# SuperScientificSoftwareLaboratory/DASP

Measured on AMD Instinct MI355X. Metric: SpMV GFLOP/s (f64), higher is better.
Workload: dtype f64; 1 GPU; HV15R synthetic stand-in (seeded; SuiteSparse dims/row statistics), A=1, x=1; rows=2017169, cols=2017169, nnz=275454726, partition=single GPU, generator_rev=26e32ff958e7, y_candidates=1

## Files before the change

### dasp_amd/_lib.py

```python
import ctypes as C
import os
import subprocess

_HERE = os.path.dirname(os.path.abspath(__file__))
SO_PATH = os.environ.get("DASP_AMD_SO") or os.path.join(_HERE, "libdasp_amd.so")


class DaspError(RuntimeError):
    def __init__(self, status, msg):
        super().__init__("dasp status %d: %s" % (status, msg))
        self.status = status


class Options(C.Structure):
    _fields_ = [
        ("threshold", C.c_double), ("block_longest", C.c_int), ("y_order", C.c_int), ("long_piece", C.c_int),
        ("host_threads", C.c_int), ("n_parts", C.c_int), ("part_bounds", C.POINTER(C.c_int)), ("part_stride", C.c_int),
        ("x_window", C.c_int), ("row_window", C.c_int), ("cid16", C.c_int), ("stream_policy", C.c_int),
        ("col_panels", C.c_int), ("slab_max_len", C.c_int), ("x_window_hybrid", C.c_int), ("piece_min_len", C.c_int),
        ("chunk_pairs", C.c_int), ("cid8", C.c_int), ("short_seg", C.c_int), ("row_tile_max", C.c_int), ("sort_columns", C.c_int),
        ("two_phase", C.c_int), ("tp_col_block", C.c_int), ("tp_row_block", C.c_int), ("long_cb", C.c_int),
        ("value_map", C.c_int),
    ]


class Stats(C.Structure):
    _fields_ = [(n, C.c_int) for n in (
        "precision rowA colA nnzA short_row_1 common_13 short_row_3 short_row_4 short_row_2 row_long row_block "
        "row_zero nnz_short nnz_long origin_nnz_reg nnz_irreg rowloop").split()] + [
        ("fill0_nnz_short", C.c_longlong), ("fill0_nnz_long", C.c_longlong), ("fill0_nnz_reg", C.c_longlong),
        ("rate_fill0", C.c_double), ("data_X", C.c_longlong), ("data_origin1", C.c_longlong),
        ("n_med_blocks", C.c_int), ("n_long_pieces", C.c_int), ("n_long_multi", C.c_int), ("n_short_tiles", C.c_int),
        ("n_workgroups", C.c_int), ("pre_ms", C.c_double),
        ("x_window_on", C.c_int), ("n_windows", C.c_int), ("n_windows_lds", C.c_int), ("lds_bytes", C.c_int),
        ("row_window", C.c_int), ("window_nnz_frac", C.c_double), ("cid16_on", C.c_int),
        ("n_col_panels", C.c_int), ("x_window_hybrid", C.c_int), ("med_rows_as_pieces", C.c_int), ("chunk_pairs", C.c_int), ("cid8_chunks", C.c_int), ("short_seg", C.c_int),
        ("row_tile_max", C.c_int), ("n_row_tiles", C.c_int), ("row_tile_nnz", C.c_longlong),
        ("two_phase", C.c_int), ("tp_col_block", C.c_int), ("tp_row_blocks", C.c_int), ("tp_units", C.c_int), ("tp_segments", C.c_longlong), ("tp_seg_elems", C.c_int),
        ("lcb_rows", C.c_int), ("lcb_col_block", C.c_int), ("lcb_units", C.c_int), ("lcb_elems", C.c_longlong),
        ("ref_fill0_nnz_short", C.c_longlong), ("ref_fill0_nnz_long", C.c_longlong), ("ref_fill0_nnz_reg", C.c_longlong), ("ref_data_X", C.c_longlong),
        ("ref_nnz_irreg", C.c_int), ("ref_origin_nnz_reg", C.c_int), ("ref_blocknum", C.c_int), ("ref_warp_number", C.c_int), ("ref_rate_fill0", C.c_double)]

    def as_dict(self):
        return {n: getattr(self, n) for n, _ in self._fields_}


class MgInfo(C.Structure):
    _fields_ = [(n, C.c_int) for n in "precision n_gpus rank rowA colA row_begin row_end stride".split()] + [
        ("nnz_own", C.c_longlong), ("nnz_other", C.c_longlong), ("overlap", C.c_int), ("has_comm", C.c_int), ("square", C.c_int), ("stream_memops", C.c_int), ("fused_step", C.c_int), ("exchange", C.c_int)]

    def as_dict(self):
        return {n: getattr(self, n) for n, _ in self._fields_}


def build(force=False):
    src = os.path.join(_HERE, "csrc")
    if force:
        subprocess.check_call(["make", "-C", src, "-s", "clean"])
    subprocess.check_call(["make", "-C", src, "-s", "-j8", "all"])
    return SO_PATH


_lib = None


def _preload_hip_runtime():
    import importlib.util
    import sys
    if "torch" in sys.modules:
        return
    try:
        spec = importlib.util.find_spec("torch")
    except (ImportError, ValueError):
        spec = None
    if spec is None or not spec.origin:
        return
    cand = os.path.join(os.path.dirname(spec.origin), "lib", "libamdhip64.so")
    if os.path.exists(cand):
        try:
            C.CDLL(cand, mode=C.RTLD_GLOBAL)
        except OSError:
            pass


def lib():
    global _lib
    if _lib is not None:
        return _lib
    if not os.path.exists(SO_PATH):
        raise ImportError(
            "dasp_amd: %s is missing. Build it with `python -c 'import __graft_entry__ as g; g.build()'` "
            "(hipcc --offload-arch=gfx950). There is no fallback implementation." % SO_PATH)
    _preload_hip_runtime()
    L = C.CDLL(SO_PATH)
    ip, vp = C.POINTER(C.c_int), C.c_void_p
    L.dasp_last_error.restype = C.c_char_p
    L.dasp_version.restype = C.c_char_p
    L.dasp_free.argtypes = [vp]
    L.dasp_options_default.argtypes = [C.POINTER(Options)]
    L.dasp_mmio_allinone_f64.argtypes = [ip, ip, ip, ip, C.POINTER(ip), C.POINTER(ip), C.POINTER(C.POINTER(C.c_double)), C.c_char_p]
    L.dasp_mmio_allinone_f16.argtypes = [ip, ip, ip, ip, C.POINTER(ip), C.POINTER(ip), C.POINTER(C.POINTER(C.c_uint16)), C.c_char_p]
    L.dasp_csr_save.argtypes = [C.c_char_p, C.c_int, C.c_int, C.c_int, C.c_int, C.c_int, vp, vp, vp]
    L.dasp_csr_load.argtypes = [C.c_char_p, C.c_int, ip, ip, ip, ip, C.POINTER(ip), C.POINTER(ip), C.POINTER(vp)]
    L.dasp_plan_create.argtypes = [C.POINTER(vp), C.c_int, C.c_int, C.c_int, C.c_int, vp, vp, vp, C.POINTER(Options)]
    L.dasp_plan_create_device.argtypes = [C.POINTER(vp), C.c_int, C.c_int, C.c_int, C.c_int, vp, vp, vp, C.POINTER(Options)]
    L.dasp_plan_download_array.argtypes = [vp, C.c_char_p, vp, C.c_size_t]
    L.dasp_plan_destroy.argtypes = [vp]
    L.dasp_plan_save.argtypes = [vp, C.c_char_p]
    L.dasp_plan_load.argtypes = [C.POINTER(vp), C.c_char_p]
    L.dasp_plan_order.argtypes = [vp]
    L.dasp_plan_order.restype = ip
    L.dasp_plan_stats.argtypes = [vp, C.POINTER(Stats)]
    L.dasp_plan_y_order.argtypes = [vp]
    L.dasp_plan_x_len.argtypes = [vp]
    L.dasp_plan_x_len.restype = C.c_longlong
    L.dasp_plan_host_array.argtypes = [vp, C.c_char_p, C.POINTER(vp), ip]
    L.dasp_plan_host_array.restype = C.c_longlong
    L.dasp_plan_panel_count.argtypes = [vp]
    L.dasp_plan_panel.argtypes = [vp, C.c_int]
    L.dasp_plan_panel.restype = vp
    L.dasp_plan_panel_range.argtypes = [vp, C.c_int, ip, ip]
    L.dasp_plan_upload.argtypes = [vp]
    L.dasp_plan_drop_host.argtypes = [vp]
    L.dasp_plan_update_values.argtypes = [vp, vp, vp]
# ... 67 lines not shown
```

### dasp_amd/api.py

```python
import ctypes as C
import os

import numpy as np

from . import _lib
from ._lib import DaspError, Options, Stats

Y_PERMUTED, Y_NATURAL = 0, 1


def _vp(a):
    return a.ctypes.data_as(C.c_void_p)


def _dtype(precision):
    if precision == 64:
        return np.float64
    if precision == 16:
        return np.float16
    raise ValueError("precision must be 64 or 16")


def mmio_allinone(filename, precision=64):
    L = _lib.lib()
    ip = C.POINTER(C.c_int)
    m, n, nnz, sym = C.c_int(), C.c_int(), C.c_int(), C.c_int()
    rp, ci = ip(), ip()
    if precision == 64:
        v = C.POINTER(C.c_double)()
        rc = L.dasp_mmio_allinone_f64(C.byref(m), C.byref(n), C.byref(nnz), C.byref(sym), C.byref(rp), C.byref(ci), C.byref(v), os.fsencode(filename))
    else:
        v = C.POINTER(C.c_uint16)()
        rc = L.dasp_mmio_allinone_f16(C.byref(m), C.byref(n), C.byref(nnz), C.byref(sym), C.byref(rp), C.byref(ci), C.byref(v), os.fsencode(filename))
    _lib.check(rc)
    k = nnz.value
    row_ptr = np.ctypeslib.as_array(rp, (m.value + 1,)).copy()
    col_idx = np.ctypeslib.as_array(ci, (max(k, 1),))[:k].copy()
    raw = np.ctypeslib.as_array(v, (max(k, 1),))[:k].copy()
    val = raw if precision == 64 else raw.view(np.float16)
    for q in (rp, ci, v):
        L.dasp_free(C.cast(q, C.c_void_p))
    return m.value, n.value, k, sym.value, row_ptr, col_idx, val


def csr_save(path, row_ptr, col_idx, val, n_cols, is_symmetric=0, precision=64):
    rp = np.ascontiguousarray(row_ptr, np.int32)
    ci = np.ascontiguousarray(col_idx, np.int32)
    v = np.ascontiguousarray(val, _dtype(precision))
    _lib.check(_lib.lib().dasp_csr_save(os.fsencode(path), precision, rp.size - 1, int(n_cols), int(ci.size), int(is_symmetric), _vp(rp), _vp(ci), _vp(v)))


def csr_load(path, precision=64):
    L = _lib.lib()
    ip = C.POINTER(C.c_int)
    m, n, nnz, sym = C.c_int(), C.c_int(), C.c_int(), C.c_int()
    rp, ci, v = ip(), ip(), C.c_void_p()
    _lib.check(L.dasp_csr_load(os.fsencode(path), precision, C.byref(m), C.byref(n), C.byref(nnz), C.byref(sym), C.byref(rp), C.byref(ci), C.byref(v)))
    k = nnz.value
    row_ptr = np.ctypeslib.as_array(rp, (m.value + 1,)).copy()
    col_idx = np.ctypeslib.as_array(ci, (max(k, 1),))[:k].copy()
    ct = C.c_double if precision == 64 else C.c_uint16
    raw = np.ctypeslib.as_array(C.cast(v, C.POINTER(ct)), (max(k, 1),))[:k].copy()
    val = raw if precision == 64 else raw.view(np.float16)
    for q in (C.cast(rp, C.c_void_p), C.cast(ci, C.c_void_p), v):
        L.dasp_free(q)
    return m.value, n.value, k, sym.value, row_ptr, col_idx, val


class Plan:

    def __init__(self, csrRowPtr, csrColIdx, csrVal, colA, precision=64, threshold=0.75, block_longest=256,
                 y_order=Y_PERMUTED, long_piece=0, host_threads=0, part_bounds=None, part_stride=0, x_window=0, row_window=0, cid16=0, stream_policy=0,
                 col_panels=0, slab_max_len=0, x_window_hybrid=0, piece_min_len=0, chunk_pairs=0, cid8=0, short_seg=0, row_tile_max=0, sort_columns=0,
                 two_phase=0, tp_col_block=0, tp_row_block=0, long_cb=0, value_map=0):
        L = _lib.lib()
        self.precision = precision
        dt = _dtype(precision)
        rp = np.ascontiguousarray(csrRowPtr, np.int32)
        ci = np.ascontiguousarray(csrColIdx, np.int32)
        v = np.ascontiguousarray(csrVal, dt)
        self.rowA, self.colA, self.nnzA = rp.size - 1, int(colA), int(ci.size)
        opt = Options()
        L.dasp_options_default(C.byref(opt))
        opt.threshold, opt.block_longest, opt.y_order = threshold, block_longest, y_order
        opt.long_piece, opt.host_threads = long_piece, host_threads
        opt.x_window, opt.row_window, opt.cid16, opt.stream_policy = x_window, row_window, cid16, stream_policy
        opt.col_panels, opt.slab_max_len, opt.x_window_hybrid, opt.piece_min_len = col_panels, slab_max_len, x_window_hybrid, piece_min_len
        opt.chunk_pairs, opt.cid8, opt.short_seg, opt.row_tile_max, opt.sort_columns = chunk_pairs, cid8, short_seg, row_tile_max, sort_columns
        opt.two_phase, opt.tp_col_block, opt.tp_row_block, opt.long_cb = two_phase, tp_col_block, tp_row_block, long_cb
        opt.value_map = value_map
        self._pb = None
        if part_bounds is not None:
            self._pb = np.ascontiguousarray(part_bounds, np.int32)
            opt.n_parts = self._pb.size - 1
            opt.part_bounds = self._pb.ctypes.data_as(C.POINTER(C.c_int))
            opt.part_stride = int(part_stride)
        self._h = C.c_void_p()
        _lib.check(L.dasp_plan_create(C.byref(self._h), precision, self.rowA, self.colA, self.nnzA, _vp(rp), _vp(ci), _vp(v), C.byref(opt)))
        self.y_order = y_order
        self.x_len = self.colA if part_bounds is None else (self._pb.size - 1) * int(part_stride)

    @classmethod
    def from_device(cls, d_row_ptr, d_col_idx, d_val, rowA, colA, nnzA, precision=64, threshold=0.75, block_longest=256,
                    y_order=Y_PERMUTED, long_piece=0, part_bounds=None, part_stride=0, x_window=0, row_window=0, cid16=0, col_panels=0, slab_max_len=0,
                    x_window_hybrid=0, piece_min_len=0, chunk_pairs=0, cid8=0, short_seg=0, row_tile_max=0, sort_columns=0, two_phase=0, tp_col_block=0, tp_row_block=0, long_cb=0,
                    value_map=0):
        L = _lib.lib()
        self = cls.__new__(cls)
        self.precision, self.rowA, self.colA, self.nnzA = precision, int(rowA), int(colA), int(nnzA)
        opt = Options()
        L.dasp_options_default(C.byref(opt))
        opt.threshold, opt.block_longest, opt.y_order, opt.long_piece = threshold, block_longest, y_order, long_piece
        opt.x_window, opt.row_window, opt.cid16, opt.col_panels = x_window, row_window, cid16, col_panels
        opt.slab_max_len, opt.x_window_hybrid, opt.piece_min_len = slab_max_len, x_window_hybrid, piece_min_len
        opt.chunk_pairs, opt.cid8, opt.short_seg, opt.row_tile_max, opt.sort_columns = chunk_pairs, cid8, short_seg, row_tile_max, sort_columns
        opt.two_phase, opt.tp_col_block, opt.tp_row_block, opt.long_cb = two_phase, tp_col_block, tp_row_block, long_cb
        opt.value_map = value_map
        self._pb = None
        if part_bounds is not None:
            self._pb = np.ascontiguousarray(part_bounds, np.int32)
            opt.n_parts, opt.part_stride = self._pb.size - 1, int(part_stride)
            opt.part_bounds = self._pb.ctypes.data_as(C.POINTER(C.c_int))
        self._h = C.c_void_p()
        _lib.check(L.dasp_plan_create_device(C.byref(self._h), precision, self.rowA, self.colA, self.nnzA, C.c_void_p(d_row_ptr),
                                             C.c_void_p(d_col_idx), C.c_void_p(d_val), C.byref(opt)))
        self.y_order = y_order
        self.x_len = int(L.dasp_plan_x_len(self._h))
        return self

    def device_array(self, name, count, dtype):
        out = np.empty(count, dtype)
        _lib.check(_lib.lib().dasp_plan_download_array(self._h, name.encode(), _vp(out), out.nbytes))
        return out

    def save(self, path):
        _lib.check(_lib.lib().dasp_plan_save(self._h, os.fsencode(path)))

    @classmethod
    def load(cls, path):
        self = cls.__new__(cls)
        self._h = C.c_void_p()
        self._pb = None
        _lib.check(_lib.lib().dasp_plan_load(C.byref(self._h), os.fsencode(path)))
        st = self.stats
        self.precision, self.rowA, self.colA, self.nnzA = st["precision"], st["rowA"], st["colA"], st["nnzA"]
        self.y_order = _lib.lib().dasp_plan_y_order(self._h)
        self.x_len = int(_lib.lib().dasp_plan_x_len(self._h))
        return self

    @property
    def order_rid(self):
        if self.rowA == 0:
            return np.zeros(0, np.int32)
        p = _lib.lib().dasp_plan_order(self._h)
        return np.ctypeslib.as_array(p, (max(self.rowA, 1),))[: self.rowA].copy()

    @property
    def stats(self):
        s = Stats()
        _lib.check(_lib.lib().dasp_plan_stats(self._h, C.byref(s)))
        return s.as_dict()

    @property
    def n_panels(self):
        return int(_lib.lib().dasp_plan_panel_count(self._h))

    def panel(self, k):
        L = _lib.lib()
        h = L.dasp_plan_panel(self._h, k)
        if not h:
            raise _lib.DaspError(-10, L.dasp_last_error().decode("utf-8", "replace"))
        b, e = C.c_int(), C.c_int()
        _lib.check(L.dasp_plan_panel_range(self._h, k, C.byref(b), C.byref(e)))
        sub = Plan.__new__(Plan)
        sub._h, sub._pb, sub._borrowed, sub._parent = C.c_void_p(h), None, True, self
        st = sub.stats
        sub.precision, sub.rowA, sub.colA, sub.nnzA = st["precision"], st["rowA"], st["colA"], st["nnzA"]
        sub.y_order, sub.x_len = Y_NATURAL, st["colA"]
        return sub, b.value, e.value

    def host_array(self, name):
        ptr, eb = C.c_void_p(), C.c_int()
        n = _lib.lib().dasp_plan_host_array(self._h, name.encode(), C.byref(ptr), C.byref(eb))
        if n < 0:
            _lib.check(int(n))
        if name in ("med_cid16", "long_cid16", "rt_start", "tp_lrow", "tp_lcol", "lcb_lcol"):
            dt = np.uint16
        elif name.endswith("_val_map"):
            dt = np.uint32
        elif name == "rt_mask":
            dt = np.uint64
        elif name == "med_cid8":
            dt = np.uint8
        elif eb.value == 4:
            dt = np.int32
        else:
            dt = np.float64 if eb.value == 8 else np.float16
        if n == 0:
            return np.zeros(0, dt)
        buf = (C.c_char * (n * eb.value)).from_address(ptr.value)
# ... 137 lines not shown
```

### dasp_amd/csrc/device.hpp

```cpp
#pragma once

#include <cstddef>
#include <vector>

#include "plan.hpp"

namespace dasp {

struct ShortDev {
    int len, count, tiles, tile0;
    long long elem_off;
    SlotMap map;
    int seg, rpt;
};

struct DevArgs {
    const void *x;
    void *y;
    const void *long_val; const int *long_cid; const int *piece_ptr; const int *piece_dst; void *partial;
    const int *multi_ptr; const int *multi_dst;
    int n_pieces, n_multi;
    int pair_mode;
    const int *med_ptr; const void *med_val; const int *med_cid;
    const unsigned short *med_cid16; const int *med_base;
    const unsigned char *med_cid8; const int *med_c8ptr;
    const int *irr_ptr; const void *irr_val; const int *irr_cid;
    int n_blocks, row_block, row_long;
    const int *med_dst; const int *win_cmin; const int *win_len;
    int n_windows, blocks_per_win;
    int win_hybrid;
    int win_xcd;
    int win_rel16;
    int ywt;
    int skip0;
    int acc;
    int wpw;
    const void *short_val; const int *short_cid; const ShortDev *groups;
    int n_short_tiles;
    int short_tpw, n_short_waves;
    int grp_wave0[kNumShortGroups];
    int grp_tile0[kNumShortGroups];
    const int *order;
    int wg_long, wg_med, wg_short;
    int xcd_on;
    int xcd_blk[9];
    int med_stride;
    const void *rt_val; const int *rt_cid; const int *rt_ptr; const unsigned short *rt_start; const unsigned long long *rt_mask;
    int n_rt_tiles, wg_rt, rt_max;
    const unsigned short *long_cid16; const int *long_base; const int *piece_c16;
    const int *med_nt;
    int wg_rot;
    int win_tiles;
};

struct TpDev {
    const unsigned short *lcol; const int *dst; const int *unit;
    const void *val; const unsigned short *lrow; void *xs;
    const int *rb_row0; const int *rb_seg0;
    int n_units, n_rb, cb, rb_max, xlen, m;
};

struct LcbDev {
    const void *val; const unsigned short *lcol; const int *ptr; const int *unit; const int *row_dst; void *partial;
    int n_units, n_rows, n_cb, cb, xlen;
};

struct ArenaMap {
    size_t long_val = 0, long_cid = 0, med_val = 0, med_cid = 0, med_cid16 = 0, med_cid8 = 0, med_base = 0, irr_val = 0, irr_cid = 0,
           short_val = 0, short_cid = 0, rt_val = 0, rt_cid = 0, long_cid16 = 0, long_base = 0, piece_c16 = 0;
};

struct DevicePlan {
    void *dargs = nullptr;
    void *args_sent = nullptr;
    void *arena = nullptr;
    size_t arena_bytes = 0;
    ArenaMap map{};
    DevArgs args{};
    TpDev tp{};
    LcbDev lcb{};
    bool nt = false;
    bool win1 = false;
    bool seven_waves = false;
    bool long16 = false;
    int device = -1;
    size_t ypart_stride = 0;
    void *vm_map = nullptr, *vm_runs = nullptr;
    bool vm_ready = false;
    void *pk_map[7] = {};
    int vm_n_runs = 0;
    long long vm_blocks = 0, vm_slots = 0;
    std::vector<Plan *> vm_arenas;
};
int value_map_upload(Plan &p);
void value_map_free(DevicePlan *d);


int require_device();
int upload_plan(Plan &p);
void choose_long16(Plan &p);
int sync_dev_args(Plan &p);
int upload_plan_unpacked(Plan &p);
int launch_spmv(Plan &p, const void *dX, void *dY, void *stream, bool accumulate);
int spmv_kernel_allow_full_lds(int precision, bool c16);
int tp_kernels_allow_lds();
int spmv_kernel_f16_resident(bool c16);
int tune_placement(Plan &p, int trials, const void *dX, void *dY, double *ms_first, double *ms_kept);

constexpr size_t kMgWordGathered = 20480, kMgWordOwnGo = 20480 + 4096, kMgWordReady = 20480 + 8192, kMgWordErr = 20480 + 12288, kMgWordXcd = 40960, kMgWordBytes = 40960 + 2048;
struct MgStepCtl {
    void *words;
    unsigned long long need;
    unsigned long long step;
    const void *mark; const void *mark_members;
    const void *blk_order;
    int n_marked, n_mark_shards;
    int max_pollers;
    int poll_sleep;
    long long timeout_ticks;
    double poll_at;
    void *err;
    int ready_by_event;
};
bool mg_step_supported(const Plan &own, const Plan *other);
void mg_step_marks(const Plan &own, const unsigned char *has_other, std::vector<unsigned char> &mark, std::vector<int> &blk_order, double hot_at = -1.0);
int launch_mg_step(Plan &own, Plan *other, const void *x_own, const void *x_gathered, void *y, const MgStepCtl &c, void *stream);
int mg_step_resident_per_cu();
struct MgStep2Ctl {
    const void *wg_list; const void *blk_order;
    int n_push, n_free, n_marked, n_total, max_pollers;
    const void *arrived; int world, rank;
    unsigned long long need;
    void *err; long long timeout_ticks; int poll_sleep;
    int fence_mode;
    void *xcd_fenced; unsigned long long step;
};
struct MgPushArgs;
int launch_mg_step2(Plan &plan, const void *x, void *y, const MgStep2Ctl &c, const MgPushArgs &push, void *stream);
int launch_mg_wait(const void *word, unsigned long long need, long long timeout_ticks, void *err, void *stream);
int launch_mg_flag(void *word, unsigned long long value, void *stream);

}
```

### dasp_amd/csrc/devpack.hip

```cpp
#include <hip/hip_runtime.h>
#include <hipcub/hipcub.hpp>

#include <memory>
#include <thread>

#include <algorithm>
#include <chrono>
#include <cstdio>
#include <cstdlib>
#include <cstring>
#include <string>
#include <type_traits>
#include <vector>

#include "device.hpp"

namespace dasp {

#define HIP_TRYP(expr)                                                                         \
    do {                                                                                       \
        hipError_t e_ = (expr);                                                                \
        if (e_ != hipSuccess) {                                                                \
            set_error(std::string(#expr) + ": " + hipGetErrorString(e_));                      \
            return e_ == hipErrorNoDevice ? DASP_ERR_NO_DEVICE : DASP_ERR_HIP;                 \
// ... 928 lines not shown
    unsigned *lmap = nullptr;
    if (p.value_map) {
        HIP_TRYP(hipMalloc(&dp.pk_map[6], L.elems * 4));
        lmap = static_cast<unsigned *>(dp.pk_map[6]);
        HIP_TRYP(hipMemset(lmap, 0, L.elems * 4));
    }
    if (s.n > 0) {
        if (vb == 8)
            hipLaunchKernelGGL((k_lcb_fill<unsigned long long>), dim3(grid_for(s.n)), dim3(256), 0, 0, s.keys, s.idx, s.n, s.start, dp.lcb.ptr, L.n_rows(), L.cb, d.ci,
                               static_cast<const unsigned long long *>(d.val), d.src, lcol, static_cast<unsigned long long *>(lval), lmap);
        else
            hipLaunchKernelGGL((k_lcb_fill<unsigned short>), dim3(grid_for(s.n)), dim3(256), 0, 0, s.keys, s.idx, s.n, s.start, dp.lcb.ptr, L.n_rows(), L.cb, d.ci,
                               static_cast<const unsigned short *>(d.val), d.src, lcol, static_cast<unsigned short *>(lval), lmap);
        HIP_TRYP(hipGetLastError());
    }
    HIP_TRYP(hipDeviceSynchronize());
    return DASP_OK;
}

int devpack_finish_two_phase(Plan &p, const DevCsr &d, const DevTiles &tp, const std::vector<long long> &off2, const std::vector<long long> &off1, const DevTiles &lcb)
{
    FormScratch sc;
    const size_t n_tiles = off1.size(), S = p.tp.segments;
    const int *d_off2 = nullptr, *d_off1 = nullptr;
    if (S > 0) {
        std::vector<int> h(off2.begin(), off2.end());
        if (int rc = form_upload(sc, h.data(), h.size(), &d_off2)) return rc;
        h.assign(off1.begin(), off1.end());
        if (int rc = form_upload(sc, h.data(), h.size(), &d_off1)) return rc;
    }
    if (int rc = upload_plan_unpacked(p)) return rc;
    DevicePlan &dp = *p.dev;
    if (S > 0) {
        auto *lcol = const_cast<unsigned short *>(dp.tp.lcol), *lrow = const_cast<unsigned short *>(dp.tp.lrow);
        auto *tval = static_cast<unsigned short *>(const_cast<void *>(dp.tp.val));
        HIP_TRYP(hipMemset(lcol, 0, S * kTpSeg * 2));
        HIP_TRYP(hipMemset(lrow, 0xFF, S * kTpSeg * 2));
        HIP_TRYP(hipMemset(tval, 0, S * kTpSeg * 2));
        unsigned *tmap = nullptr;
        if (p.value_map) {
            HIP_TRYP(hipMalloc(&dp.pk_map[5], S * kTpSeg * 4));
            tmap = static_cast<unsigned *>(dp.pk_map[5]);
            HIP_TRYP(hipMemset(tmap, 0, S * kTpSeg * 4));
        }
        const int n_cb = std::max(1, (p.n + p.tp.cb - 1) / p.tp.cb);
        if (tp.n > 0) hipLaunchKernelGGL(k_tp_fill, dim3(grid_for(tp.n)), dim3(256), 0, 0, tp.keys, tp.idx, tp.n, tp.start, d_off2, d_off1, n_cb, p.tp.cb, d.ci,
                                         static_cast<const unsigned short *>(d.val), d.src, lcol, lrow, tval, tmap);
        HIP_TRYP(hipGetLastError());
        hipLaunchKernelGGL(k_tp_dst, dim3(grid_for((long long)S)), dim3(256), 0, 0, d_off2, d_off1, (int)n_tiles, (int)S, const_cast<int *>(dp.tp.dst));
        HIP_TRYP(hipGetLastError());
    }
    if (int rc = lcb_fill(p, d, lcb)) return rc;
    HIP_TRYP(hipDeviceSynchronize());
    p.host_dropped = true;
    if (p.value_map) return value_map_upload(p);
    return DASP_OK;
}

int devpack_finish_panels_lcb(Plan &p, const DevCsr &d, const DevTiles &lcb)
{
    if (int rc = upload_plan_unpacked(p)) return rc;
    if (int rc = lcb_fill(p, d, lcb)) return rc;
    p.host_dropped = true;
    if (p.value_map) return value_map_upload(p);
    return DASP_OK;
}

int devpack_finish_panels(Plan &p) { return upload_plan(p); }
int devpack_fetch_csr(const Plan &p, const DevCsr &d, int *ci, void *val)
{
    if (p.nnz <= 0) return DASP_OK;
    HIP_TRYP(hipMemcpy(ci, d.ci, (size_t)p.nnz * sizeof(int), hipMemcpyDeviceToHost));
    if (val) HIP_TRYP(hipMemcpy(val, d.val, (size_t)p.nnz * (size_t)p.geo.vbytes, hipMemcpyDeviceToHost));
    return DASP_OK;
}
int devpack_current_device() { int d = 0; if (hipGetDevice(&d) != hipSuccess) { (void)hipGetLastError(); d = 0; } return d; }
void devpack_use_device(int device) { if (device >= 0) (void)hipSetDevice(device); }

int devpack_all(Plan &p, const DevCsr &d, const PackMeta &m)
{
    if (int rc = upload_plan_unpacked(p)) return rc;
    const int rc = p.precision == 64 ? pack_all_typed<double>(p, d, m) : pack_all_typed<_Float16>(p, d, m);
    if (rc == DASP_OK) p.host_dropped = true;
    if (rc == DASP_OK && p.value_map && !p.panel) return value_map_upload(p);
    return rc;
}

__global__ void k_spin_us(long long ticks)
{
    const long long t0 = wall_clock64();
    while (wall_clock64() - t0 < ticks) __builtin_amdgcn_s_sleep(8);
}
__global__ void __launch_bounds__(256) k_spin_fat(long long ticks, int *sink)
{
    __shared__ int pad[19744 / 4];
    asm volatile("v_mov_b32 v255, 0" ::: "v255");
    asm volatile("v_accvgpr_write_b32 a23, 0" ::: "a23");
    pad[threadIdx.x] = (int)ticks;
    const long long t0 = wall_clock64();
    while (wall_clock64() - t0 < ticks) __builtin_amdgcn_s_sleep(8);
    if (ticks < 0) sink[threadIdx.x] = pad[255 - threadIdx.x];
}
int devpack_spin(void *stream, int micros, int channels)
{
    if (micros <= 0) return DASP_OK;
    if (channels > 0) hipLaunchKernelGGL(k_spin_fat, dim3(channels), dim3(256), 0, static_cast<hipStream_t>(stream), (long long)micros * 100, (int *)nullptr);
    else hipLaunchKernelGGL(k_spin_us, dim3(1), dim3(64), 0, static_cast<hipStream_t>(stream), (long long)micros * 100);
    HIP_TRYP(hipGetLastError());
    return DASP_OK;
}

namespace {

struct ValueRun { long long dst_off, map_off, count, blk0; int arena, pad; };
constexpr int kRefreshMaxArenas = 65;
constexpr int kRefreshThreads = 256, kRefreshSteps = 4;
struct RefreshBases { char *base[kRefreshMaxArenas]; };
template <int VB> struct RefreshGeo { static constexpr int G = VB == 8 ? 4 : 8; };
__host__ __device__ constexpr long long refresh_slots_per_block(int vb) { return (long long)kRefreshThreads * kRefreshSteps * (vb == 8 ? 4 : 8); }

typedef unsigned int vm_u32x4 __attribute__((ext_vector_type(4)));
typedef unsigned long long vm_u64x2 __attribute__((ext_vector_type(2)));

template <class V, bool NT> __device__ __forceinline__ V vm_load(const V *p) { if constexpr (NT) return __builtin_nontemporal_load(p); else return *p; }
template <class V, bool NT> __device__ __forceinline__ void vm_store(V *p, V v) { if constexpr (NT) __builtin_nontemporal_store(v, p); else *p = v; }

template <int VB, bool NT>
__global__ void __launch_bounds__(kRefreshThreads) dasp_value_refresh_kernel(const ValueRun *__restrict__ runs, int n_runs, const unsigned int *__restrict__ map,
                                                                           const void *__restrict__ src, RefreshBases bases)
{
    using W = std::conditional_t<VB == 8, unsigned long long, unsigned short>;
    constexpr int G = RefreshGeo<VB>::G;
    const long long b = blockIdx.x;
    int lo = 0, hi = n_runs - 1;
    while (lo < hi) { const int mid = (lo + hi + 1) >> 1; if (runs[mid].blk0 <= b) lo = mid; else hi = mid - 1; }
    const long long count = runs[lo].count, e_blk = (b - runs[lo].blk0) * refresh_slots_per_block(VB);
    W *dst = reinterpret_cast<W *>(bases.base[runs[lo].arena] + runs[lo].dst_off);
    const unsigned int *mp = map + runs[lo].map_off;
    const W *s = static_cast<const W *>(src);
#pragma unroll
    for (int step = 0; step < kRefreshSteps; ++step) {
        const long long e = e_blk + ((long long)step * kRefreshThreads + threadIdx.x) * G;
        if (e + G <= count) {
            unsigned int ix[G];
            const vm_u32x4 m0 = vm_load<vm_u32x4, NT>(reinterpret_cast<const vm_u32x4 *>(mp + e));
            ix[0] = m0.x; ix[1] = m0.y; ix[2] = m0.z; ix[3] = m0.w;
            if constexpr (G == 8) {
                const vm_u32x4 m1 = vm_load<vm_u32x4, NT>(reinterpret_cast<const vm_u32x4 *>(mp + e + 4));
                ix[4] = m1.x; ix[5] = m1.y; ix[6] = m1.z; ix[7] = m1.w;
            }
            W v[G];
#pragma unroll
            for (int i = 0; i < G; ++i) v[i] = ix[i] ? s[ix[i] - 1u] : (W)0;
            if constexpr (VB == 8) {
                vm_store<vm_u64x2, NT>(reinterpret_cast<vm_u64x2 *>(dst + e), vm_u64x2{v[0], v[1]});
                vm_store<vm_u64x2, NT>(reinterpret_cast<vm_u64x2 *>(dst + e + 2), vm_u64x2{v[2], v[3]});
            } else {
                vm_u32x4 o;
                o.x = (unsigned)v[0] | ((unsigned)v[1] << 16); o.y = (unsigned)v[2] | ((unsigned)v[3] << 16);
                o.z = (unsigned)v[4] | ((unsigned)v[5] << 16); o.w = (unsigned)v[6] | ((unsigned)v[7] << 16);
                vm_store<vm_u32x4, NT>(reinterpret_cast<vm_u32x4 *>(dst + e), o);
            }
        } else if (e < count) {
            for (long long j = e; j < count; ++j) { const unsigned int ix = mp[j]; dst[j] = ix ? s[ix - 1u] : (W)0; }
        }
    }
}
// ... 112 lines not shown
    const char *s = static_cast<const char *>(val);
    const int T = resolve_threads(p.opt.host_threads);
    for (const HostRun &r : hr) {
        char *dst = r.host_val->data();
        const uint32_t *mp = r.map->data();
        const size_t n = r.count, per = std::max<size_t>(1 << 16, (n + (size_t)T - 1) / (size_t)T);
        std::vector<std::thread> th;
        auto work = [&](size_t b, size_t e) {
            for (size_t j = b; j < e; ++j) { if (mp[j]) std::memcpy(dst + j * vb, s + (size_t)(mp[j] - 1) * vb, vb); else std::memset(dst + j * vb, 0, vb); }
        };
        for (size_t b = per; b < n; b += per) th.emplace_back(work, b, std::min(n, b + per));
        work(0, std::min(n, per));
        for (auto &t : th) t.join();
    }
}

static int value_map_usable(const Plan &p)
{
    if (p.panel) { set_error("a column panel is refreshed through its parent plan (dasp_plan_update_values on the parent)"); return DASP_ERR_ARG; }
    if (p.loaded) { set_error("a plan loaded from a file carries no value map (plan files do not store one): create the plan with value_map = 1"); return DASP_ERR_STATE; }
    if (!p.value_map) { set_error("the plan has no value map: create it with dasp_options_t::value_map = 1"); return DASP_ERR_STATE; }
    return DASP_OK;
}

}

extern "C" {

int dasp_plan_update_values(dasp_plan_t *plan, const void *dVal, void *stream)
{
    using namespace dasp;
    if (!plan || (!dVal && plan->impl.nnz > 0)) { set_error("dasp_plan_update_values: NULL argument"); return DASP_ERR_ARG; }
    Plan &p = plan->impl;
    if (int rc = value_map_usable(p)) return rc;
    if (!p.dev) { set_error("dasp_plan_update_values: the plan is not uploaded (dasp_plan_upload, or dasp_plan_update_values_host for host values)"); return DASP_ERR_STATE; }
    if (!p.dev->vm_ready) { set_error("dasp_plan_update_values: the plan's value map did not reach the device (its upload failed): upload the plan again"); return DASP_ERR_STATE; }
    if (!p.host_dropped) if (int rc = dasp_plan_drop_host(plan)) return rc;
    return value_refresh_launch(p, dVal, static_cast<hipStream_t>(stream));
}

int dasp_plan_update_values_host(dasp_plan_t *plan, const void *csrVal)
{
    using namespace dasp;
    if (!plan || (!csrVal && plan->impl.nnz > 0)) { set_error("dasp_plan_update_values_host: NULL argument"); return DASP_ERR_ARG; }
    Plan &p = plan->impl;
    if (int rc = value_map_usable(p)) return rc;
    if (p.dev && !p.dev->vm_ready) { set_error("dasp_plan_update_values_host: the plan's value map did not reach the device (its upload failed): upload the plan again"); return DASP_ERR_STATE; }
    try {
        if (!p.host_dropped) value_refresh_host(p, csrVal);
    } catch (const std::exception &e) { set_error(std::string("dasp_plan_update_values_host: ") + e.what()); return DASP_ERR_NOMEM; }
    if (p.dev && p.dev->vm_blocks > 0) {
        const size_t bytes = (size_t)p.nnz * (size_t)p.geo.vbytes;
        void *stage = nullptr;
        HIP_TRYP(hipDeviceSynchronize());
        HIP_TRYP(hipMalloc(&stage, std::max<size_t>(bytes, 16)));
        hipError_t e = hipMemcpy(stage, csrVal, bytes, hipMemcpyHostToDevice);
        int rc = e == hipSuccess ? value_refresh_launch(p, stage, nullptr) : DASP_ERR_HIP;
        if (e != hipSuccess) set_error(std::string("dasp_plan_update_values_host: staging copy: ") + hipGetErrorString(e));
        if (rc == DASP_OK && (e = hipStreamSynchronize(nullptr)) != hipSuccess) { set_error(std::string("dasp_plan_update_values_host: ") + hipGetErrorString(e)); rc = DASP_ERR_HIP; }
        (void)hipFree(stage);
        return rc;
    }
    return DASP_OK;
}

long long dasp_plan_value_map_slots(const dasp_plan_t *plan)
{
    using namespace dasp;
    if (!plan) return DASP_ERR_ARG;
    const Plan &p = plan->impl;
    if (!p.value_map || p.loaded) return 0;
    if (p.host_dropped) return p.dev ? p.dev->vm_slots : 0;
    std::vector<HostRun> hr;
    collect_runs(const_cast<Plan &>(p), hr);
    long long n = 0;
    for (const HostRun &r : hr) n += (long long)r.count;
    return n;
}

}

namespace dasp {

int download_array(Plan &p, const char *name, void *dst, size_t bytes)
{
    if (!p.dev || !p.dev->arena) { set_error("plan not on the device"); return DASP_ERR_STATE; }
    const ArenaMap &mp = p.dev->map;
    const size_t vb = (size_t)p.geo.vbytes;
    if (std::strcmp(name, "lcb_val") == 0 && p.dev->lcb.val) {
        if (bytes != p.lcb.elems * vb) { set_error("size mismatch for lcb_val"); return DASP_ERR_ARG; }
        if (bytes) HIP_TRYP(hipMemcpy(dst, p.dev->lcb.val, bytes, hipMemcpyDeviceToHost));
        return DASP_OK;
    }
    if (std::strcmp(name, "lcb_lcol") == 0 && p.dev->lcb.lcol) {
        if (bytes != p.lcb.elems * 2) { set_error("size mismatch for lcb_lcol"); return DASP_ERR_ARG; }
        if (bytes) HIP_TRYP(hipMemcpy(dst, p.dev->lcb.lcol, bytes, hipMemcpyDeviceToHost));
        return DASP_OK;
    }
    if (p.two_phase) {
        const TpDev &q = p.dev->tp;
        const size_t S = p.tp.segments;
        struct { const char *n; const void *ptr; size_t len; } tt[] = {
            {"tp_lcol", q.lcol, S * kTpSeg * 2}, {"tp_dst", q.dst, S * 4}, {"tp_val", q.val, S * kTpSeg * vb}, {"tp_lrow", q.lrow, S * kTpSeg * 2}, {"tp_xs", q.xs, S * kTpSeg * vb}};
        for (auto &t : tt)
            if (std::strcmp(t.n, name) == 0) {
                if (bytes != t.len) { set_error(std::string("size mismatch for ") + name); return DASP_ERR_ARG; }
                if (t.len) HIP_TRYP(hipMemcpy(dst, t.ptr, t.len, hipMemcpyDeviceToHost));
                return DASP_OK;
            }
        set_error(std::string("unknown device array of a two-phase plan: ") + name);
        return DASP_ERR_ARG;
    }
    struct { const char *n; size_t off, len; } tab[] = {
        {"long_val", mp.long_val, p.cnt_long * vb}, {"long_cid", mp.long_cid, p.cnt_long * 4}, {"long_cid16", mp.long_cid16, p.cnt_long * 2}, {"long_base", mp.long_base, p.cnt_long_chunks * 4},
        {"med_val", mp.med_val, p.cnt_reg * vb}, {"med_cid", mp.med_cid, p.cid16 ? 0 : p.cnt_reg * 4},
        {"med_cid16", mp.med_cid16, p.cid16 ? (p.cnt_reg - p.cnt_reg8) * 2 : 0}, {"med_cid8", mp.med_cid8, p.cnt_reg8}, {"med_base", mp.med_base, p.cid16 ? (size_t)p.med_ptr.back() * 4 : 0},
        {"irr_val", mp.irr_val, p.cnt_irr * vb}, {"irr_cid", mp.irr_cid, p.cnt_irr * 4},
        {"short_val", mp.short_val, p.cnt_short * vb}, {"short_cid", mp.short_cid, p.cnt_short * 4},
        {"rt_val", mp.rt_val, p.cnt_rt * vb}, {"rt_cid", mp.rt_cid, p.cnt_rt * 4},
    };
    for (auto &t : tab)
        if (std::strcmp(t.n, name) == 0) {
            if (bytes != t.len) { set_error(std::string("size mismatch for ") + name); return DASP_ERR_ARG; }
            if (t.len) HIP_TRYP(hipMemcpy(dst, static_cast<char *>(p.dev->arena) + t.off, t.len, hipMemcpyDeviceToHost));
            return DASP_OK;
        }
    set_error(std::string("unknown device array: ") + name);
    return DASP_ERR_ARG;
}

}
```

### dasp_amd/csrc/kernels.hip

```cpp
#include <hip/hip_runtime.h>

#include <chrono>
#include <thread>
#include <cmath>
#include <cstdint>
#include <cstdio>
#include <cstdlib>
#include <cstring>
#include <string>
#include <vector>

#include "plan.hpp"
#include "device.hpp"

#include "spmv_device.hpp"

namespace dasp {
#ifdef DASP_STAMPS
extern int g_stamp_launch;
#endif

template <class T, bool NT, bool C16, bool WIN, bool C8 = false, int MW = 0, bool L16 = false>
__global__ __launch_bounds__(WIN ? 1024 : 256, WIN ? kMinWavesWin : MW ? MW : kMinWavesPlain) void dasp_spmv_kernel(CallArgs c)
{
    extern __shared__ __attribute__((aligned(16))) char lds_raw[];
#ifdef DASP_STAMPS
    Stamps st; st.begin(c.stamp_launch);
#else
    Stamps st; st.begin(0);
#endif
    const DevArgs a = load_args(c);
    static_assert(!L16 || (!WIN && !C8 && MW == 0), "the 16-bit long ids ride in the plain build only");
    spmv_body<T, NT, C16, WIN, C8, false, WIN, L16>(a, lds_raw, blockIdx.x, st);
#ifdef DASP_STAMPS
    st.finish(a.wpw);
#endif
}

template <class T, bool NT, bool C16>
__global__ __launch_bounds__(256, sizeof(T) == 2 ? 7 : kMinWavesPlain) void dasp_spmv_rt_kernel(CallArgs c)
{
    extern __shared__ __attribute__((aligned(16))) char lds_raw[];
#ifdef DASP_STAMPS
    Stamps st; st.begin(c.stamp_launch);
#else
    Stamps st; st.begin(0);
#endif
    const DevArgs a = load_args(c);
    spmv_body<T, NT, C16, false, false, true>(a, lds_raw, blockIdx.x, st);
}

template <class T, bool C16>
__global__ __launch_bounds__(1024, 4) void dasp_spmv_win1_kernel(CallArgs c)
{
    extern __shared__ __attribute__((aligned(16))) char lds_raw[];
#ifdef DASP_STAMPS
    Stamps st; st.begin(c.stamp_launch);
#else
    Stamps st; st.begin(0);
#endif
    const DevArgs a = load_args(c);
    spmv_body<T, true, C16, true, false>(a, lds_raw, blockIdx.x, st);
#ifdef DASP_STAMPS
    st.finish(a.wpw);
#endif
}

constexpr int kMaxMergedPanels = 8;
struct PanelCall {
    const DevArgs *plan[kMaxMergedPanels];
    int wg_end[kMaxMergedPanels];
    const void *x; char *part; size_t stride_bytes; int np;
};
__device__ __forceinline__ CallArgs panel_of(const PanelCall &c, int &wg)
{
    int k = 0, first = 0;
    const DevArgs *p = c.plan[0];
#pragma unroll
    for (int i = 1; i < kMaxMergedPanels; ++i) {
        const bool in = i < c.np && (int)blockIdx.x >= c.wg_end[i - 1];
        k = in ? i : k; first = in ? c.wg_end[i - 1] : first; p = in ? c.plan[i] : p;
    }
    wg = (int)blockIdx.x - first;
#ifdef DASP_STAMPS
    return CallArgs{p, c.x, c.part + (size_t)k * c.stride_bytes, 0, 0, -1};
#else
    return CallArgs{p, c.x, c.part + (size_t)k * c.stride_bytes, 0, 0};
#endif
}
template <class T, bool NT, bool C16>
__global__ __launch_bounds__(256, sizeof(T) == 2 ? 7 : kMinWavesPlain) void dasp_spmv_panels_kernel(PanelCall c)
{
    extern __shared__ __attribute__((aligned(16))) char lds_raw[];
    int wg;
    const CallArgs ca = panel_of(c, wg);
    Stamps st; st.begin(0);
    const DevArgs a = load_args(ca);
    spmv_body<T, NT, C16, false, false, true>(a, lds_raw, wg, st);
}

template <class T>
__global__ __launch_bounds__(256) void dasp_long_reduce_kernel(CallArgs c)
{
    const DevArgs a = load_args(c);
    using part_t = typename Tr<T>::part_t;
    __shared__ part_t wsum[kWavesPerWG];
    const int lane = threadIdx.x & 63, wave = threadIdx.x >> 6;
    const int i = blockIdx.x;
    const int q0 = a.multi_ptr[i], q1 = a.multi_ptr[i + 1];
    const part_t *part = static_cast<const part_t *>(a.partial);
    part_t s0 = 0, s1 = 0, s2 = 0, s3 = 0;
    int q = q0 + (int)threadIdx.x;
    for (; q + 768 < q1; q += 1024) { s0 += part[q]; s1 += part[q + 256]; s2 += part[q + 512]; s3 += part[q + 768]; }
    for (; q < q1; q += 256) s0 += part[q];
    const part_t s = wave_sum((s0 + s1) + (s2 + s3));
    if (lane == 0) wsum[wave] = s;
// ... 233 lines not shown
    acc = __builtin_amdgcn_mfma_f64_16x16x4f64(A, B, acc, 0, 0, 0);
    for (int r = 0; r < 4; ++r) D[((l >> 4) + 4 * r) * 16 + (l & 15)] = acc[r];
}
__global__ void selftest_f16_kernel(float *D)
{
    const int l = threadIdx.x;
    f16x4 A, B;
    for (int j = 0; j < 4; ++j) {
        const int k = 4 * (l >> 4) + j;
        A[j] = (_Float16)(float)(((l & 15) + 2 * k) % 7 + 1);
        B[j] = (_Float16)(float)((3 * k + (l & 15)) % 5 + 1);
    }
    f32x4 acc = {0, 0, 0, 0};
    acc = __builtin_amdgcn_mfma_f32_16x16x16f16(A, B, acc, 0, 0, 0);
    for (int r = 0; r < 4; ++r) D[(4 * (l >> 4) + r) * 16 + (l & 15)] = acc[r];
}


#define HIP_TRY(expr)                                                                          \
    do {                                                                                       \
        hipError_t e_ = (expr);                                                                \
        if (e_ != hipSuccess) {                                                                \
            set_error(std::string(#expr) + ": " + hipGetErrorString(e_));                      \
            return e_ == hipErrorNoDevice ? DASP_ERR_NO_DEVICE : DASP_ERR_HIP;                 \
        }                                                                                      \
    } while (0)


int spmv_kernel_allow_full_lds(int precision, bool c16)
{
    const int bytes = kWinLdsMax;
    hipError_t e1, e2;
#define DASP_ATTR(TT, NTV, CV) hipFuncSetAttribute(reinterpret_cast<const void *>(&dasp_spmv_kernel<TT, NTV, CV, true>), hipFuncAttributeMaxDynamicSharedMemorySize, bytes)
    if (precision == 64) { e1 = c16 ? DASP_ATTR(double, true, true) : DASP_ATTR(double, true, false); e2 = c16 ? DASP_ATTR(double, false, true) : DASP_ATTR(double, false, false); }
    else { e1 = c16 ? DASP_ATTR(_Float16, true, true) : DASP_ATTR(_Float16, true, false); e2 = c16 ? DASP_ATTR(_Float16, false, true) : DASP_ATTR(_Float16, false, false); }
#undef DASP_ATTR
    HIP_TRY(e1);
    HIP_TRY(e2);
    if (precision == 64) HIP_TRY(c16 ? hipFuncSetAttribute(reinterpret_cast<const void *>(&dasp_spmv_win1_kernel<double, true>), hipFuncAttributeMaxDynamicSharedMemorySize, bytes)
                                     : hipFuncSetAttribute(reinterpret_cast<const void *>(&dasp_spmv_win1_kernel<double, false>), hipFuncAttributeMaxDynamicSharedMemorySize, bytes));
    else HIP_TRY(c16 ? hipFuncSetAttribute(reinterpret_cast<const void *>(&dasp_spmv_win1_kernel<_Float16, true>), hipFuncAttributeMaxDynamicSharedMemorySize, bytes)
                     : hipFuncSetAttribute(reinterpret_cast<const void *>(&dasp_spmv_win1_kernel<_Float16, false>), hipFuncAttributeMaxDynamicSharedMemorySize, bytes));
    return DASP_OK;
}
int spmv_kernel_f16_resident(bool c16)
{
    const void *fn = c16 ? reinterpret_cast<const void *>(&dasp_spmv_kernel<_Float16, true, true, false>)
                         : reinterpret_cast<const void *>(&dasp_spmv_kernel<_Float16, true, false, false>);
    int fit = 0;
    if (hipOccupancyMaxActiveBlocksPerMultiprocessor(&fit, fn, kWave * kWavesPerWG, 0) != hipSuccess) fit = 0;
    (void)hipGetLastError();
    return fit;
}

template <class T>
static int launch_typed(Plan &p, const DevArgs &a, hipStream_t s)
{
    const int grid = a.wg_long + a.wg_med + a.wg_short + a.wg_rt;
    const bool nt = p.dev->nt;
    if (int rc = sync_dev_args(p)) return rc;
#ifdef DASP_STAMPS
    const CallArgs c{static_cast<const DevArgs *>(p.dev->dargs), a.x, a.y, a.acc, a.ywt, g_stamp_launch >= 0 ? g_stamp_launch++ : -1};
#else
    const CallArgs c{static_cast<const DevArgs *>(p.dev->dargs), a.x, a.y, a.acc, a.ywt};
#endif
    if (a.wg_rt > 0) {
        const size_t lds = (size_t)kWavesPerWG * kRowTile * (size_t)a.rt_max * sizeof(typename Tr<T>::part_t);
        if (nt && p.cid16) hipLaunchKernelGGL((dasp_spmv_rt_kernel<T, true, true>), dim3(grid), dim3(256), lds, s, c);
        else if (nt) hipLaunchKernelGGL((dasp_spmv_rt_kernel<T, true, false>), dim3(grid), dim3(256), lds, s, c);
        else if (p.cid16) hipLaunchKernelGGL((dasp_spmv_rt_kernel<T, false, true>), dim3(grid), dim3(256), lds, s, c);
        else hipLaunchKernelGGL((dasp_spmv_rt_kernel<T, false, false>), dim3(grid), dim3(256), lds, s, c);
    } else if (grid > 0) {
        const size_t lds = p.windowed ? (size_t)p.lds_bytes : 0;
        const bool c16 = p.cid16;
#define DASP_FOR_EACH(M) \
        if (nt && c16 && p.windowed) { M(true, true, true); } else if (nt && c16) { M(true, true, false); } \
        else if (nt && p.windowed) { M(true, false, true); } else if (nt) { M(true, false, false); } \
        else if (c16 && p.windowed) { M(false, true, true); } else if (c16) { M(false, true, false); } \
        else if (p.windowed) { M(false, false, true); } else { M(false, false, false); }
#define DASP_LAUNCH(NTV, CV, WINV) hipLaunchKernelGGL((dasp_spmv_kernel<T, NTV, CV, WINV>), dim3(grid), dim3(kWave * a.wpw), lds, s, c)
        if (p.windowed && p.dev->win1 && !nt) {
            if (c16) hipLaunchKernelGGL((dasp_spmv_win1_kernel<T, true>), dim3(grid), dim3(kWave * a.wpw), lds, s, c);
            else hipLaunchKernelGGL((dasp_spmv_win1_kernel<T, false>), dim3(grid), dim3(kWave * a.wpw), lds, s, c);
        } else if (sizeof(T) == 8 && c16 && !p.windowed && p.cnt_reg8 > 0) {
            if (p.dev->seven_waves) {
                if (nt) hipLaunchKernelGGL((dasp_spmv_kernel<double, true, true, false, true, 7>), dim3(grid), dim3(kWave * a.wpw), lds, s, c);
                else hipLaunchKernelGGL((dasp_spmv_kernel<double, false, true, false, true, 7>), dim3(grid), dim3(kWave * a.wpw), lds, s, c);
            }
            else if (nt) hipLaunchKernelGGL((dasp_spmv_kernel<double, true, true, false, true>), dim3(grid), dim3(kWave * a.wpw), lds, s, c);
            else hipLaunchKernelGGL((dasp_spmv_kernel<double, false, true, false, true>), dim3(grid), dim3(kWave * a.wpw), lds, s, c);
        } else if (!p.windowed && p.dev->long16 && !(sizeof(T) == 8 && p.dev->seven_waves)) {
            if (nt && c16) hipLaunchKernelGGL((dasp_spmv_kernel<T, true, true, false, false, 0, true>), dim3(grid), dim3(kWave * a.wpw), lds, s, c);
            else if (nt) hipLaunchKernelGGL((dasp_spmv_kernel<T, true, false, false, false, 0, true>), dim3(grid), dim3(kWave * a.wpw), lds, s, c);
            else if (c16) hipLaunchKernelGGL((dasp_spmv_kernel<T, false, true, false, false, 0, true>), dim3(grid), dim3(kWave * a.wpw), lds, s, c);
            else hipLaunchKernelGGL((dasp_spmv_kernel<T, false, false, false, false, 0, true>), dim3(grid), dim3(kWave * a.wpw), lds, s, c);
        } else if (sizeof(T) == 8 && !p.windowed && p.dev->seven_waves) {
            if (nt && c16) hipLaunchKernelGGL((dasp_spmv_kernel<double, true, true, false, false, 7>), dim3(grid), dim3(kWave * a.wpw), lds, s, c);
            else if (nt) hipLaunchKernelGGL((dasp_spmv_kernel<double, true, false, false, false, 7>), dim3(grid), dim3(kWave * a.wpw), lds, s, c);
            else if (c16) hipLaunchKernelGGL((dasp_spmv_kernel<double, false, true, false, false, 7>), dim3(grid), dim3(kWave * a.wpw), lds, s, c);
            else hipLaunchKernelGGL((dasp_spmv_kernel<double, false, false, false, false, 7>), dim3(grid), dim3(kWave * a.wpw), lds, s, c);
        } else
        DASP_FOR_EACH(DASP_LAUNCH)
#undef DASP_LAUNCH
#undef DASP_FOR_EACH
    }
    if (a.n_multi > 0)
        hipLaunchKernelGGL((dasp_long_reduce_kernel<T>), dim3(a.n_multi), dim3(256), 0, s, c);
    HIP_TRY(hipGetLastError());
    return DASP_OK;
}

int set_stream_policy(Plan &p, int policy)
{
    if (policy < 0 || policy > 2) { set_error("stream_policy must be 0, 1 or 2"); return DASP_ERR_ARG; }
    p.opt.stream_policy = policy;
    if (p.dev) p.dev->nt = policy == 2 || (policy != 1 && p.stats.data_X > kStreamBytes);
    const int sub = policy != 0 ? policy : (p.stats.data_X > kStreamBytes ? 2 : 1);
    for (auto &h : p.panels) if (int rc = set_stream_policy(h->impl, sub)) return rc;
    return DASP_OK;
}

int tp_kernels_allow_lds()
{
    HIP_TRY(hipFuncSetAttribute(reinterpret_cast<const void *>(&dasp_tp_expand_kernel<_Float16>), hipFuncAttributeMaxDynamicSharedMemorySize, 160 * 1024));
    HIP_TRY(hipFuncSetAttribute(reinterpret_cast<const void *>(&dasp_tp_reduce_kernel<_Float16>), hipFuncAttributeMaxDynamicSharedMemorySize, 160 * 1024));
    HIP_TRY(hipFuncSetAttribute(reinterpret_cast<const void *>(&dasp_lcb_kernel<_Float16>), hipFuncAttributeMaxDynamicSharedMemorySize, 160 * 1024));
    HIP_TRY(hipFuncSetAttribute(reinterpret_cast<const void *>(&dasp_lcb_kernel<double>), hipFuncAttributeMaxDynamicSharedMemorySize, 160 * 1024));
    return DASP_OK;
}

template <class T>
static int launch_panels_merged_typed(Plan &p, const void *dX, char *part, size_t stride_bytes, hipStream_t s)
{
    const int np = (int)p.panels.size();
    PanelCall c{}, r{};
    c.x = dX; c.part = part; c.stride_bytes = stride_bytes; c.np = np;
    int grid = 0, grid2 = 0, rt_max = 0;
    const Plan &p0 = p.panels[0]->impl;
    for (int k = 0; k < np; ++k) {
        Plan &q = p.panels[(size_t)k]->impl;
        if (!q.dev || !q.dev->arena || q.windowed || q.two_phase || !q.panels.empty() || q.cnt_reg8 > 0 || q.cid16 != p0.cid16 || q.dev->nt != p0.dev->nt || q.dev->args.med_stride != p0.dev->args.med_stride) return 1;
        if (int rc = sync_dev_args(q)) return rc;
        const DevArgs &a = q.dev->args;
        grid += a.wg_long + a.wg_med + a.wg_short + a.wg_rt;
        grid2 += (a.n_multi + kWavesPerWG - 1) / kWavesPerWG;
        rt_max = std::max(rt_max, a.wg_rt > 0 ? a.rt_max : 0);
        c.plan[k] = static_cast<const DevArgs *>(q.dev->dargs); c.wg_end[k] = grid;
        r.plan[k] = c.plan[k]; r.wg_end[k] = grid2;
    }
    r.x = dX; r.part = part; r.stride_bytes = stride_bytes; r.np = np;
    const size_t lds = (size_t)kWavesPerWG * kRowTile * (size_t)rt_max * sizeof(typename Tr<T>::part_t);
    const bool nt = p0.dev->nt, c16 = p0.cid16;
    if (grid > 0) {
        if (nt && c16) hipLaunchKernelGGL((dasp_spmv_panels_kernel<T, true, true>), dim3(grid), dim3(256), lds, s, c);
        else if (nt) hipLaunchKernelGGL((dasp_spmv_panels_kernel<T, true, false>), dim3(grid), dim3(256), lds, s, c);
        else if (c16) hipLaunchKernelGGL((dasp_spmv_panels_kernel<T, false, true>), dim3(grid), dim3(256), lds, s, c);
        else hipLaunchKernelGGL((dasp_spmv_panels_kernel<T, false, false>), dim3(grid), dim3(256), lds, s, c);
    }
    if (grid2 > 0) hipLaunchKernelGGL((dasp_long_reduce_panels_kernel<T>), dim3(grid2), dim3(256), 0, s, r);
    HIP_TRY(hipGetLastError());
    return DASP_OK;
}
static int launch_panels_merged(Plan &p, const void *dX, char *part, size_t stride_bytes, hipStream_t s)
{
    static const bool off = [] { const char *e = std::getenv("DASP_PANELS_MERGED"); return e && std::atoi(e) == 0; }();
    if (off || p.panels.empty() || p.panels.size() > (size_t)kMaxMergedPanels) return 1;
// ... 195 lines not shown
```

### dasp_amd/csrc/multigpu.cpp

```cpp
#include <hip/hip_runtime_api.h>
#include <hip/hip_ext.h>
#include <rccl/rccl.h>

#include <dlfcn.h>

#include <algorithm>
#include <chrono>
#include <cstdlib>
#include <cstring>
#include <exception>
#include <memory>
#include <mutex>
#include <new>
#include <string>
#include <thread>
#include <vector>

#include <unistd.h>

#include "plan.hpp"
#include "device.hpp"
#include "mgx.hpp"

using namespace dasp;
// ... 187 lines not shown
    std::vector<void *> fake_peers;
    ncclComm_t comm = nullptr;

    size_t vb() const { return precision == 64 ? 8 : 2; }
    size_t all_bytes() const { return (size_t)stride * vb() * (size_t)world; }
    bool one_stream() const { return step2 && fused && push; }
    char *gcur() const { return static_cast<char *>(yg) + (one_stream() ? (size_t)(k2 & 1) * all_bytes() : push ? (size_t)(xseq & 1) * all_bytes() : 0); }
    int rows() const { return bounds[(size_t)rank + 1] - bounds[(size_t)rank]; }
    ~dasp_mg_plan()
    {
        if (device >= 0) (void)hipSetDevice(device);
        if (cs) (void)hipStreamSynchronize(cs);
        if (device >= 0) (void)hipDeviceSynchronize();
        if (comm && rccl()->CommDestroy) (void)rccl()->CommDestroy(comm);
        for (size_t r = 0; r < peer_opened.size(); ++r)
            if (peer_opened[r]) { if (peer_gather[r]) (void)hipIpcCloseMemHandle(peer_gather[r]); if (peer_flags[r]) (void)hipIpcCloseMemHandle(peer_flags[r]); }
        for (void *p : {xflags, d_push_dst, d_push_count, push_scratch, d_wg_list, d_push_dst2, d_push_count2}) if (p) (void)hipFree(p);
        if (ev_y) (void)hipEventDestroy(ev_y);
        if (ev_g) (void)hipEventDestroy(ev_g);
        for (hipEvent_t e : ev_x) if (e) (void)hipEventDestroy(e);
        if (err_word) (void)hipHostFree(err_word);
        if (cs) (void)hipStreamDestroy(cs);
        if (rs) (void)hipStreamDestroy(rs);
        for (uint64_t *w : sig) if (w) (void)hipFree(w);
        if (words) (void)hipFree(words);
        if (d_mark) (void)hipFree(d_mark);
        if (d_blk_order) (void)hipFree(d_blk_order);
        for (void *p : {ys[0], yg}) if (p) (void)hipFree(p);
        if (xg && xg != yg) (void)hipFree(xg);
        if (own) dasp_plan_destroy(own);
        if (other) dasp_plan_destroy(other);
    }
};

namespace {

template <class T>
void split_by_owner(int m, const int *rp, const int *ci, const T *val, int lo, int hi, int threads,
                    std::vector<int> &rpO, std::vector<int> &ciO, std::vector<T> &vO,
                    std::vector<int> &rpR, std::vector<int> &ciR, std::vector<T> &vR)
{
    rpO.assign((size_t)m + 1, 0); rpR.assign((size_t)m + 1, 0);
    auto par = [&](auto f) {
        const int parts = std::max(1, std::min(threads, m / 4096 + 1));
        std::vector<std::thread> th;
        for (int t = 0; t < parts; ++t) {
            const int b = (int)((long long)m * t / parts), e = (int)((long long)m * (t + 1) / parts);
            th.emplace_back([=] { f(b, e); });
        }
        for (auto &x : th) x.join();
    };
    par([&](int b, int e) {
        for (int i = b; i < e; ++i) {
            int o = 0;
            for (int j = rp[i]; j < rp[i + 1]; ++j) o += ci[j] >= lo && ci[j] < hi;
            rpO[(size_t)i + 1] = o; rpR[(size_t)i + 1] = rp[i + 1] - rp[i] - o;
        }
    });
    for (int i = 0; i < m; ++i) { rpO[(size_t)i + 1] += rpO[i]; rpR[(size_t)i + 1] += rpR[i]; }
    ciO.resize((size_t)rpO[m]); vO.resize((size_t)rpO[m]); ciR.resize((size_t)rpR[m]); vR.resize((size_t)rpR[m]);
    par([&](int b, int e) {
        for (int i = b; i < e; ++i) {
            int o = rpO[i], r = rpR[i];
            for (int j = rp[i]; j < rp[i + 1]; ++j) {
                if (ci[j] >= lo && ci[j] < hi) { ciO[(size_t)o] = ci[j] - lo; vO[(size_t)o++] = val[j]; }
                else { ciR[(size_t)r] = ci[j]; vR[(size_t)r++] = val[j]; }
            }
        }
    });
}

template <class T>
int create_impl(dasp_mg_plan &g, const int *rp, const int *ci, const T *val, const dasp_options_t *user)
{
    const int m = g.rows();
    const int lo = g.bounds[(size_t)g.rank], hi = g.bounds[(size_t)g.rank + 1];
    dasp_options_t opt;
    if (user) opt = *user; else dasp_options_default(&opt);
    opt.y_order = DASP_Y_NATURAL;
    opt.short_seg = -1;
    opt.two_phase = -1;
    opt.n_parts = 0; opt.part_bounds = nullptr; opt.part_stride = 0;
    opt.value_map = 0;
    const int nnz = rp[m];
    if (!g.square) {
        g.nnz_own = nnz; g.nnz_other = 0;
        return dasp_plan_create(&g.own, g.precision, m, g.colA, nnz, rp, ci, val, &opt);
    }
    dasp_options_t part = opt;
    part.n_parts = g.world; part.part_bounds = g.bounds.data(); part.part_stride = g.stride;
    if (!g.overlap) {
        g.nnz_own = nnz; g.nnz_other = 0;
        return dasp_plan_create(&g.own, g.precision, m, g.colA, nnz, rp, ci, val, &part);
    }
    if (g.step2) {
        std::vector<unsigned char> has((size_t)std::max(m, 1), 0);
        long long other = 0;
        for (int i = 0; i < m; ++i) {
            int o = 0;
            for (int j = rp[i]; j < rp[i + 1]; ++j) o += !(ci[j] >= lo && ci[j] < hi);
            has[(size_t)i] = o > 0; other += o;
        }
        g.nnz_own = nnz - other; g.nnz_other = other;
        if (int rc = dasp_plan_create(&g.own, g.precision, m, g.colA, nnz, rp, ci, val, &part)) return rc;
        const Plan &P = g.own->impl;
        if (g.precision == 64 && P.panels.empty() && !P.windowed && P.opt.y_order == DASP_Y_NATURAL) {
            double hot_at = 1.0;
            if (const char *e = std::getenv("DASP_MG_HOT_AT")) hot_at = std::max(0.0, std::min(1.0, std::atof(e)));
            mg_step_marks(P, has.data(), g.mark, g.blk_order, hot_at);
            const int n_pieces = (int)P.piece_dst.size(), wg_long = (n_pieces + kWavesPerWG - 1) / kWavesPerWG;
            const int wg_med = (P.stats.n_med_blocks + kWavesPerWG - 1) / kWavesPerWG;
            int first_hot_med = wg_long + wg_med;
            for (int w = wg_long; w < wg_long + wg_med; ++w) if (g.mark[(size_t)w]) { first_hot_med = w; break; }
            g.wg_list.clear(); g.wg_list.reserve(g.mark.size());
            for (int w = 0; w < first_hot_med; ++w) if (!g.mark[(size_t)w]) g.wg_list.push_back(w);
            g.n_free2 = (int)g.wg_list.size();
            for (size_t w = 0; w < g.mark.size(); ++w) if (g.mark[w]) g.wg_list.push_back((int)w);
            g.n_marked2 = (int)g.wg_list.size() - g.n_free2;
            for (int w = first_hot_med; w < (int)g.mark.size(); ++w) if (!g.mark[(size_t)w]) g.wg_list.push_back(w);
        }
        return DASP_OK;
    }
    std::vector<int> rpO, ciO, rpR, ciR;
    std::vector<T> vO, vR;
    split_by_owner<T>(m, rp, ci, val, lo, hi, resolve_threads(opt.host_threads), rpO, ciO, vO, rpR, ciR, vR);
    g.nnz_own = rpO[(size_t)m]; g.nnz_other = rpR[(size_t)m];
    static const int zero = 0;
    if (int rc = dasp_plan_create(&g.own, g.precision, m, g.stride, rpO[(size_t)m], rpO.data(), ciO.empty() ? &zero : ciO.data(),
                                  vO.empty() ? static_cast<const void *>(&zero) : vO.data(), &opt)) return rc;
    if (part.cid16 == 0 && g.precision == 64 && g.own->impl.cid16) part.cid16 = 1;
    if (g.nnz_other > 0)
        if (int rc = dasp_plan_create(&g.other, g.precision, m, g.colA, rpR[(size_t)m], rpR.data(), ciR.data(), vR.data(), &part)) return rc;
    if (g.other && g.precision == 64 && g.own->impl.panels.empty() && !g.own->impl.windowed && g.own->impl.opt.y_order == DASP_Y_NATURAL) {
        std::vector<unsigned char> has((size_t)std::max(m, 1), 0);
        for (int i = 0; i < m; ++i) has[(size_t)i] = rpR[(size_t)i + 1] > rpR[(size_t)i];
        mg_step_marks(g.own->impl, has.data(), g.mark, g.blk_order);
        g.mark_members.assign(64, 0);
        for (size_t w = 0; w < g.mark.size(); ++w) if (g.mark[w]) { ++g.mark_members[w & 63]; ++g.n_marked; }
        for (unsigned c : g.mark_members) g.n_mark_shards += c > 0;
    }
    return DASP_OK;
}

constexpr uint64_t kAllBits = 0xFFFFFFFFFFFFFFFFull;
constexpr int kExchangeKernelRegs = 288;
int handoff_ready(dasp_mg_plan &g, hipStream_t s, uint64_t k)
{
    if (g.use_sig) {
        if (hipStreamWriteValue64(s, g.sig[0], k, 0) == hipSuccess &&
            hipStreamWaitValue64(g.cs, g.sig[0], k, hipStreamWaitValueGte, kAllBits) == hipSuccess) return DASP_OK;
        (void)hipGetLastError(); g.use_sig = false;
    }
    MG_HIP(hipEventRecord(g.ev_y, s));
    MG_HIP(hipStreamWaitEvent(g.cs, g.ev_y, 0));
    return DASP_OK;
}
int publish_gathered(dasp_mg_plan &g, uint64_t k)
{
    g.pending_sig = false;
    if (g.use_sig) {
        if (hipStreamWriteValue64(g.cs, g.sig[1], k, 0) == hipSuccess) { g.pending_sig = true; return DASP_OK; }
        (void)hipGetLastError(); g.use_sig = false;
    }
    MG_HIP(hipEventRecord(g.ev_g, g.cs));
    return DASP_OK;
}
// ... 740 lines not shown
```

### dasp_amd/csrc/planio.cpp

```cpp
#include <algorithm>
#include <cstdio>
#include <cstring>
#include <string>

#include "plan.hpp"

namespace dasp {

namespace {
const char kPlanMagic[8] = {'D', 'A', 'S', 'P', 'P', 'L', 'N', '8'};

struct Writer {
    FILE *f; bool ok = true;
    void raw(const void *p, size_t n) { if (ok && n && std::fwrite(p, 1, n, f) != n) ok = false; }
    template <class V> void vec(const V &v) { long long b = (long long)(v.size() * sizeof(typename V::value_type)); raw(&b, 8); raw(v.data(), (size_t)b); }
};
struct Reader {
    FILE *f; long long left; bool ok = true;
    void raw(void *p, size_t n)
    {
        if (!ok || !n) return;
        if ((long long)n > left || std::fread(p, 1, n, f) != n) { ok = false; return; }
        left -= (long long)n;
    }
    template <class V> void vec(V &v)
    {
        long long b = -1; raw(&b, 8);
        if (!ok || b < 0 || b > left || b % (long long)sizeof(typename V::value_type)) { ok = false; return; }
        v.resize((size_t)b / sizeof(typename V::value_type));
        raw(v.data(), (size_t)b);
    }
};

template <class IO> void arrays(IO &io, Plan &p)
{
    io.vec(p.part_bounds); io.vec(p.order); io.vec(p.dst_map); io.vec(p.panel_bounds);
    io.vec(p.long_val); io.vec(p.long_cid); io.vec(p.long_cid16); io.vec(p.long_base); io.vec(p.piece_c16); io.vec(p.piece_ptr); io.vec(p.piece_dst); io.vec(p.multi_ptr); io.vec(p.multi_dst);
    io.vec(p.med_ptr); io.vec(p.med_val); io.vec(p.med_cid); io.vec(p.med_cid16); io.vec(p.med_cid8); io.vec(p.med_c8ptr); io.vec(p.med_korig); io.vec(p.med_base);
    io.vec(p.irr_ptr); io.vec(p.irr_val); io.vec(p.irr_cid);
    io.vec(p.med_dst); io.vec(p.win_cmin); io.vec(p.win_len);
    io.vec(p.short_val); io.vec(p.short_cid);
    io.vec(p.rt_ptr); io.vec(p.rt_start); io.vec(p.rt_mask); io.vec(p.rt_val); io.vec(p.rt_cid);
    io.vec(p.tp.rb_row0); io.vec(p.tp.rb_seg0); io.vec(p.tp.unit); io.vec(p.tp.dst); io.vec(p.tp.lcol); io.vec(p.tp.lrow); io.vec(p.tp.val);
    io.vec(p.lcb.row_dst); io.vec(p.lcb.row_id); io.vec(p.lcb.ptr); io.vec(p.lcb.unit); io.vec(p.lcb.lcol); io.vec(p.lcb.val);
}
}

static bool validate_plan(const Plan &p, int n_panels, bool is_panel, std::string &why)
{
    auto fail = [&](const char *w) { why = w; return false; };
    const Geometry geo = p.geo;
    const long long vb = geo.vbytes, CH = geo.chunk, SR = geo.short_rows;
    const long long m = p.m;
    if (p.m < 0 || p.n < 0 || p.nnz < 0) return fail("negative dimension");
    if (p.opt.y_order != DASP_Y_PERMUTED && p.opt.y_order != DASP_Y_NATURAL) return fail("y_order");
    if (p.opt.n_parts < 0 || p.opt.n_parts > (1 << 20) || (p.opt.n_parts > 0 && p.opt.part_stride <= 0)) return fail("column partition");
    if (p.opt.n_parts > 0) {
        if (p.part_bounds.size() != (size_t)p.opt.n_parts + 1 || p.part_bounds.front() != 0 || p.part_bounds.back() != p.n) return fail("part_bounds size / span");
        for (int g = 0; g < p.opt.n_parts; ++g)
            if (p.part_bounds[g + 1] < p.part_bounds[g] || p.part_bounds[g + 1] - p.part_bounds[g] > p.opt.part_stride) return fail("part_bounds not monotone or wider than part_stride");
    } else if (!p.part_bounds.empty()) return fail("part_bounds without n_parts");
    const long long xlen = p.opt.n_parts > 0 ? (long long)p.opt.n_parts * p.opt.part_stride : (long long)p.n;
    if (xlen >= (1ll << 31)) return fail("x length");
    if (p.order.size() != (size_t)m) return fail("order size");
    {
        std::vector<bool> seen((size_t)m, false);
        for (int v : p.order) {
            if ((unsigned)v >= (unsigned)m) return fail("order_rid entry out of range");
            if (seen[(size_t)v]) return fail("order_rid is not a permutation: two writers for one y index in natural order");
            seen[(size_t)v] = true;
        }
    }
    if (!p.dst_map.empty()) {
        if (p.dst_map.size() != (size_t)m) return fail("dst_map size");
        for (int v : p.dst_map) if ((unsigned)v >= (unsigned)m) return fail("dst_map entry out of range");
    }
    if (p.stats.rowA != p.m || p.stats.colA != p.n || p.stats.nnzA != p.nnz || p.stats.precision != p.precision) return fail("stats header");
    if (p.stats.row_long < 0 || p.n_mfma_rows < 0 || p.n_mfma_rows > p.stats.row_block || (long long)p.stats.row_long + p.stats.row_block > m) return fail("category counters");
    if (n_panels == 0 && (p.med_slot0 < p.stats.row_long || (long long)p.med_slot0 + p.n_mfma_rows > (long long)p.stats.row_long + p.stats.row_block)) return fail("med_slot0");
    if (p.panel_bounds.size() != 2 * (size_t)n_panels) return fail("panel_bounds size");
    if (p.two_phase) {
        if (n_panels > 0 || is_panel) return fail("two-phase plan with column panels");
        if (p.cnt_long || p.cnt_reg || p.cnt_irr || p.cnt_short || p.cnt_rt || !p.med_ptr.empty() || !p.irr_ptr.empty() || !p.piece_ptr.empty()) return fail("two-phase plan holds packed DASP arrays");
        if (!validate_two_phase(p, why)) return false;
// ... 108 lines not shown
            if (len == 0 || p.win_hybrid) continue;
            for (long long b = w * bpw; b < std::min(nb, (w + 1) * bpw); ++b) {
                for (long long c = p.med_ptr[(size_t)b]; c < p.med_ptr[(size_t)b + 1]; ++c)
                    for (long long e = 0; e < CH; ++e) {
                        const long long col = cid_at(b, c, e);
                        if (col < 0) continue;
                        if (col < c0 || col >= c0 + len) return fail("windowed column id outside its LDS span");
                    }
                for (long long r = b * kMedRows; r < std::min<long long>(p.n_mfma_rows, (b + 1) * kMedRows); ++r)
                    for (int t = p.irr_ptr[(size_t)r]; t < p.irr_ptr[(size_t)r + 1]; ++t) { const int col = p.irr_cid[(size_t)t]; if (col >= 0 && (col < c0 || col >= c0 + len)) return fail("windowed tail id outside its LDS span"); }
            }
        }
    } else if (!p.med_dst.empty() || !p.win_len.empty() || !p.win_cmin.empty()) return fail("window tables without windows");
    if (p.short_val.size() != p.cnt_short * (size_t)vb || p.short_cid.size() != p.cnt_short || !cid_ok(p.short_cid)) return fail("short arrays");
    long long off = 0, tile0 = 0;
    static const int kLen[5] = {1, 2, 3, 4, 0};
    for (int g = 0; g < kNumShortGroups; ++g) {
        const ShortGroup &G = p.grp[g];
        if (G.len != (g < 5 ? kLen[g] : g) || G.count < 0 || G.count > m) return fail("short group length / count");
        const bool seg_ok = G.seg == 0 || (G.seg == 1 && G.len >= 1 && G.len <= 4 && !p.windowed);
        if (!seg_ok || G.rpt != (G.seg ? short_seg_rows(G.len) : (int)SR)) return fail("short group layout");
        if (G.tiles != (G.count + G.rpt - 1) / G.rpt || G.tile0 != tile0 || G.elem_off != off) return fail("short group tiles / offsets");
        tile0 += G.tiles; off += (long long)G.tiles * short_tile_elems(G.seg != 0, G.len, (int)SR);
        const SlotMap &M = G.map;
        if (M.split < 0 || M.grp[0] < 0 || M.grp[1] < 0) return fail("slot map");
        for (int t : {0, M.split - 1, M.split, G.count - 1})
            if (t >= 0 && t < G.count) { const long long sl = M.slot(t); if (sl < 0 || sl >= m) return fail("slot map leaves the permutation"); }
    }
    if ((size_t)off != p.cnt_short || p.stats.n_short_tiles != tile0) return fail("short segment size");
    if (p.rt_max == 0) { if (!p.rt_ptr.empty() || !p.rt_start.empty() || !p.rt_mask.empty() || p.cnt_rt) return fail("row tiles without rt_max"); }
    else {
        const size_t tiles = (size_t)((m + kRowTile - 1) / kRowTile);
        if (p.rt_max < 0 || p.rt_max > kRowTileMax || !is_panel || p.windowed || p.cnt_reg8) return fail("row tiles: bound / not a plain column panel");
        if (p.rt_mask.size() != tiles || p.rt_ptr.size() != tiles + 1 || p.rt_start.size() != tiles * kRowTile || !mono(p.rt_ptr) || (size_t)p.rt_ptr.back() != p.cnt_rt)
            return fail("row tile tables");
        if (p.rt_val.size() != p.cnt_rt * (size_t)vb || p.rt_cid.size() != p.cnt_rt) return fail("row tile arrays");
        for (int v : p.rt_cid) if (v < 0 || v >= xlen) return fail("row tile column id out of range");
        for (size_t t = 0; t < tiles; ++t) {
            const int n = p.rt_ptr[t + 1] - p.rt_ptr[t];
            for (int i = 0; i < kRowTile; ++i) {
                const int s = p.rt_start[t * kRowTile + (size_t)i], e = i + 1 < kRowTile ? p.rt_start[t * kRowTile + (size_t)i + 1] : n;
                const bool on = (p.rt_mask[t] >> i) & 1;
                if ((i == 0 && s != 0) || e < s || e > n || e - s > p.rt_max || (!on && e != s) || (on && (long long)t * kRowTile + i >= m)) return fail("row tile row table");
            }
        }
    }
    if (p.win_hybrid && !p.windowed) return fail("win_hybrid without windows");
    if (p.win_rel16) {
        if (!p.windowed || !p.cid16 || p.win_hybrid) return fail("win_rel16 needs LDS windows with 16-bit ids");
        const long long bpw = p.row_window / kMedRows;
        for (long long b = 0; b < nb; ++b) {
            const size_t w = (size_t)(b / bpw);
            if (p.win_len[w] <= 0) continue;
            if (p.win_len[w] > 65534) return fail("win_rel16: staged span beyond 16-bit offsets");
            for (long long c = p.med_ptr[(size_t)b]; c < p.med_ptr[(size_t)b + 1]; ++c)
                if (p.med_base[(size_t)c] != p.win_cmin[w]) return fail("win_rel16: a chunk base differs from its window's first staged column");
        }
    }
    {
        const bool natural = p.opt.y_order == DASP_Y_NATURAL;
        std::vector<bool> hit((size_t)m, false);
        auto claim = [&](long long yi) { if (yi < 0 || yi >= m || hit[(size_t)yi]) return false; hit[(size_t)yi] = true; return true; };
        auto ydst = [&](long long slot) -> long long {
            if (slot < 0 || slot >= m) return -1;
            if (!natural) return slot;
            const int r = p.order[(size_t)slot];
            return p.dst_map.empty() ? r : p.dst_map[(size_t)r];
        };
        for (size_t t = 0; t < p.rt_mask.size(); ++t)
            for (int i = 0; i < kRowTile; ++i) if (((p.rt_mask[t] >> i) & 1) && !claim((long long)t * kRowTile + i)) return fail("two writers for one y index (row tiles)");
        for (int d : p.piece_dst) if (d >= 0 && !claim(d)) return fail("two writers for one y index (piece_dst)");
        for (int d : p.multi_dst) if (!claim(d)) return fail("two writers for one y index (multi_dst)");
        for (long long r = 0; r < p.n_mfma_rows; ++r)
            if (!claim(p.windowed ? (long long)p.med_dst[(size_t)r] : ydst((long long)p.med_slot0 + r))) return fail("two writers for one y index (medium rows)");
        for (int g = 0; g < kNumShortGroups; ++g) {
            if (is_panel && p.grp[g].len == 0) continue;
            for (int t = 0; t < p.grp[g].count; ++t)
                if (!claim(ydst(g < 5 ? (long long)p.grp[g].map.slot(t) : (long long)p.grp[g].map.base[0] + t))) return fail("two writers for one y index (short rows / slabs)");
        }
    }
    return true;
}

static void write_plan(Writer &w, Plan &p)
{
    const int hdr[25] = {p.precision, p.m, p.n, p.nnz, p.opt.y_order, p.windowed ? 1 : 0, p.row_window, p.lds_bytes, p.cid16 ? 1 : 0,
                         p.opt.n_parts, p.opt.part_stride, p.opt.stream_policy, (int)p.panels.size(), p.n_mfma_rows, p.win_hybrid ? 1 : 0, p.med_slot0, p.pair_mode, p.win_rel16 ? 1 : 0, p.rt_max,
                         p.two_phase ? 1 : 0, p.tp.cb, p.tp.rb_max, p.lcb.cb, p.lcb.n_cb, p.lcb.h};
    w.raw(hdr, sizeof hdr); w.raw(&p.stats, sizeof p.stats); w.raw(p.grp, sizeof p.grp);
    arrays(w, p);
    for (auto &h : p.panels) write_plan(w, h->impl);
}

static bool read_plan(Reader &r, Plan &p, int depth, std::string &r_why)
{
    int hdr[25];
    r.raw(hdr, sizeof hdr);
    if (!r.ok || (hdr[0] != 64 && hdr[0] != 16) || hdr[12] < 0 || hdr[12] > 64 || (depth > 0 && hdr[12] != 0)) return false;
    p.precision = hdr[0]; p.geo = geometry_for(p.precision);
    p.m = hdr[1]; p.n = hdr[2]; p.nnz = hdr[3];
    dasp_options_default(&p.opt);
    p.opt.y_order = hdr[4]; p.windowed = hdr[5] != 0; p.row_window = hdr[6]; p.lds_bytes = hdr[7]; p.cid16 = hdr[8] != 0;
    p.opt.n_parts = hdr[9]; p.opt.part_stride = hdr[10]; p.opt.stream_policy = hdr[11]; p.n_mfma_rows = hdr[13]; p.win_hybrid = hdr[14] != 0; p.med_slot0 = hdr[15]; p.pair_mode = hdr[16]; p.win_rel16 = hdr[17] != 0; p.rt_max = hdr[18];
    if (p.pair_mode < 0 || p.pair_mode > 2 || (p.windowed && p.pair_mode)) return false;
    p.two_phase = hdr[19] != 0; p.tp.cb = hdr[20]; p.tp.rb_max = hdr[21];
    p.lcb.cb = hdr[22]; p.lcb.n_cb = hdr[23]; p.lcb.h = hdr[24];
    if (p.two_phase && (depth > 0 || hdr[12] != 0)) return false;
    r.raw(&p.stats, sizeof p.stats); r.raw(p.grp, sizeof p.grp);
    arrays(r, p);
    if (!r.ok) return false;
    p.tp.segments = p.tp.dst.size();
    p.lcb.elems = p.lcb.lcol.size();
    p.opt.two_phase = p.two_phase ? 1 : -1; p.opt.tp_col_block = p.tp.cb; p.opt.tp_row_block = p.tp.rb_max;
    p.opt.part_bounds = p.part_bounds.empty() ? nullptr : p.part_bounds.data();
    const size_t vb = (size_t)p.geo.vbytes;
    const int np = hdr[12];
    bool sane = p.m >= 0 && p.order.size() == (size_t)p.m && p.stats.rowA == p.m && p.stats.precision == p.precision &&
                (p.dst_map.empty() || p.dst_map.size() == (size_t)p.m) && p.panel_bounds.size() == 2 * (size_t)np &&
                p.long_val.size() == p.long_cid.size() * vb && p.irr_val.size() == p.irr_cid.size() * vb &&
                p.short_val.size() == p.short_cid.size() * vb &&
                (p.cid16 ? p.med_val.size() == (p.med_cid16.size() + p.med_cid8.size()) * vb : p.med_val.size() == p.med_cid.size() * vb);
    if (np == 0 && !p.two_phase)
        sane = sane && p.piece_ptr.size() == p.piece_dst.size() + 1 && p.irr_ptr.size() == (size_t)p.n_mfma_rows + 1 &&
               p.n_mfma_rows >= 0 && p.n_mfma_rows <= p.stats.row_block && (!p.windowed || p.med_dst.size() == (size_t)p.n_mfma_rows);
    if (!sane) return false;
    p.cnt_long = p.long_cid.size(); p.cnt_irr = p.irr_cid.size(); p.cnt_short = p.short_cid.size();
    p.cnt_long_chunks = p.long_base.size();
    p.cnt_reg = p.cid16 ? p.med_cid16.size() + p.med_cid8.size() : p.med_cid.size();
    p.cnt_reg8 = p.med_cid8.size();
    p.cnt_rt = p.rt_cid.size();
    p.host_dropped = false;
    p.loaded = true;
    p.panel = depth > 0;
    if (!validate_plan(p, np, depth > 0, r_why)) return false;
    p.opt.col_panels = np > 0 ? np : 1;
    for (int k = 0; k < np; ++k) {
        std::unique_ptr<dasp_plan> h(new dasp_plan());
        if (!read_plan(r, h->impl, depth + 1, r_why) || h->impl.m != p.m || h->impl.precision != p.precision) return false;
        p.panels.push_back(std::move(h));
    }
    if (np > 0) {
        long long have = 0;
        for (const auto &h : p.panels) have += (long long)h->impl.nnz + (long long)h->impl.cnt_rt;
        for (uint16_t c : p.lcb.lcol) have += c != kLcbPadCol;
        if (have != p.nnz) { r_why = "the panels and the column-blocked long rows do not add up to nnzA"; return false; }
    }
    return true;
}

int save_plan(Plan &p, const char *path)
{
    if (!path) return DASP_ERR_ARG;
    if (p.host_dropped) { set_error("host arrays were dropped: nothing to save"); return DASP_ERR_STATE; }
    FILE *f = std::fopen(path, "wb");
    if (!f) { set_error(std::string("cannot create ") + path); return DASP_ERR_OPEN; }
    Writer w{f};
    w.raw(kPlanMagic, 8);
    const int abi[3] = {(int)sizeof(dasp_stats_t), kNumShortGroups, (int)sizeof(ShortGroup)};
    w.raw(abi, sizeof abi);
    write_plan(w, p);
    const bool ok = (std::fclose(f) == 0) && w.ok;
    if (!ok) { set_error(std::string("short write to ") + path); return DASP_ERR_OPEN; }
    return DASP_OK;
}

int load_plan(Plan &p, const char *path)
{
    if (!path) return DASP_ERR_ARG;
    FILE *f = std::fopen(path, "rb");
    if (!f) { set_error(std::string("cannot open ") + path); return DASP_ERR_OPEN; }
    std::fseek(f, 0, SEEK_END);
    const long long size = std::ftell(f);
    std::fseek(f, 0, SEEK_SET);
    Reader r{f, size < 0 ? 0 : size};
    char magic[8];
    int abi[3] = {0, 0, 0};
    r.raw(magic, 8);
    r.raw(abi, sizeof abi);
    if (!r.ok || std::memcmp(magic, kPlanMagic, 8) != 0 || abi[0] != (int)sizeof(dasp_stats_t) || abi[1] != kNumShortGroups || abi[2] != (int)sizeof(ShortGroup)) {
        std::fclose(f); set_error("not a DASPPLN7 plan file of this build (magic / struct sizes differ)"); return DASP_ERR_BANNER;
    }
    std::string why;
    bool ok = false;
    try { ok = read_plan(r, p, 0, why); }
    catch (...) { std::fclose(f); throw; }
    std::fclose(f);
    if (!ok) { set_error("truncated or inconsistent plan file" + (why.empty() ? std::string() : ": " + why)); return DASP_ERR_ENTRY; }
    return DASP_OK;
}

}
```

### dasp_amd/csrc/spmv_device.hpp

```cpp
#pragma once
#include <hip/hip_runtime.h>

#include <cstdint>

#include "plan.hpp"
#include "device.hpp"

namespace dasp {

typedef double f64x4 __attribute__((ext_vector_type(4)));
typedef double f64x2 __attribute__((ext_vector_type(2)));
typedef float f32x4 __attribute__((ext_vector_type(4)));
typedef _Float16 f16x4 __attribute__((ext_vector_type(4)));
typedef int i32x4 __attribute__((ext_vector_type(4)));
typedef int i32x2 __attribute__((ext_vector_type(2)));
typedef unsigned short u16x4 __attribute__((ext_vector_type(4)));
typedef unsigned short u16x8 __attribute__((ext_vector_type(8)));
typedef const __attribute__((address_space(1))) unsigned char *gbyte_p;
typedef _Float16 f16x8 __attribute__((ext_vector_type(8)));


template <bool NT, class U>
__device__ __forceinline__ U ldg(const U *p)
{
    if constexpr (NT) return __builtin_nontemporal_load(p);
    else return *p;
}

template <int CTRL>
__device__ __forceinline__ double dpp_mov_f64(double v)
{
    int lo = __double2loint(v), hi = __double2hiint(v);
    lo = __builtin_amdgcn_update_dpp(lo, lo, CTRL, 0xf, 0xf, false);
    hi = __builtin_amdgcn_update_dpp(hi, hi, CTRL, 0xf, 0xf, false);
    return __hiloint2double(hi, lo);
}
template <int CTRL>
__device__ __forceinline__ float dpp_mov_f32(float v)
{
    return __int_as_float(__builtin_amdgcn_update_dpp(__float_as_int(v), __float_as_int(v), CTRL, 0xf, 0xf, false));
}
__device__ __forceinline__ double readlane_f64(double v, int l)
{
    int lo = __builtin_amdgcn_readlane(__double2loint(v), l);
    int hi = __builtin_amdgcn_readlane(__double2hiint(v), l);
    return __hiloint2double(hi, lo);
}
__device__ __forceinline__ double wave_sum(double v)
{
    v += dpp_mov_f64<0x128>(v);
    v += dpp_mov_f64<0x124>(v);
    v += dpp_mov_f64<0x122>(v);
    v += dpp_mov_f64<0x121>(v);
    return (readlane_f64(v, 0) + readlane_f64(v, 16)) + (readlane_f64(v, 32) + readlane_f64(v, 48));
}
__device__ __forceinline__ float wave_sum(float v)
{
    v += dpp_mov_f32<0x128>(v);
    v += dpp_mov_f32<0x124>(v);
    v += dpp_mov_f32<0x122>(v);
    v += dpp_mov_f32<0x121>(v);
    float a = __int_as_float(__builtin_amdgcn_readlane(__float_as_int(v), 0));
    float b = __int_as_float(__builtin_amdgcn_readlane(__float_as_int(v), 16));
    float c = __int_as_float(__builtin_amdgcn_readlane(__float_as_int(v), 32));
    float d = __int_as_float(__builtin_amdgcn_readlane(__float_as_int(v), 48));
    return (a + b) + (c + d);
}

template <bool K, class U>
__device__ __forceinline__ U tab(const U *p, int i)
{
    if constexpr (K) return reinterpret_cast<const __attribute__((address_space(4))) U *>(reinterpret_cast<uintptr_t>(p))[i];
    else return p[i];
}

#ifdef DASP_STAMPS
struct CallArgs { const DevArgs *plan; const void *x; void *y; int acc, ywt, stamp_launch; };
#else
struct CallArgs { const DevArgs *plan; const void *x; void *y; int acc, ywt; };
#endif
template <class U> __device__ __forceinline__ U *ldp(U *const *field)
{
    typedef __attribute__((address_space(1))) U *gptr;
    return (U *)*reinterpret_cast<const __attribute__((address_space(4))) gptr *>(reinterpret_cast<uintptr_t>(field));
}
__device__ __forceinline__ DevArgs load_args(const CallArgs &c)
{
    static_assert(sizeof(DevArgs) % 4 == 0, "DevArgs is a whole number of words");
    int w[sizeof(DevArgs) / 4];
#pragma unroll
    for (int i = 0; i < (int)(sizeof(DevArgs) / 4); ++i) w[i] = tab<true>(reinterpret_cast<const int *>(c.plan), i);
    DevArgs a;
    __builtin_memcpy(&a, w, sizeof a);
#define DASP_G(f) a.f = ldp(&c.plan->f)
    DASP_G(long_val); DASP_G(long_cid); DASP_G(long_cid16); DASP_G(long_base); DASP_G(piece_c16); DASP_G(piece_ptr); DASP_G(piece_dst); DASP_G(partial); DASP_G(multi_ptr); DASP_G(multi_dst);
    DASP_G(med_ptr); DASP_G(med_val); DASP_G(med_cid); DASP_G(med_cid16); DASP_G(med_base); DASP_G(med_cid8); DASP_G(med_c8ptr);
    DASP_G(irr_ptr); DASP_G(med_nt); DASP_G(irr_val); DASP_G(irr_cid); DASP_G(med_dst); DASP_G(win_cmin); DASP_G(win_len);
    DASP_G(short_val); DASP_G(short_cid); DASP_G(groups); DASP_G(order);
    DASP_G(rt_val); DASP_G(rt_cid); DASP_G(rt_ptr); DASP_G(rt_start); DASP_G(rt_mask);
#undef DASP_G
    a.x = c.x; a.y = c.y; a.acc = c.acc; a.ywt = c.ywt;
    return a;
}

template <int I, int N> struct LastLE {
    static __device__ __forceinline__ void run(const int (&arr)[N], int w, int &idx, int &val)
    {
        if constexpr (I < N) { const bool in = w >= arr[I]; idx = in ? I : idx; val = in ? arr[I] : val; LastLE<I + 1, N>::run(arr, w, idx, val); }
    }
};
template <int I, int N> struct PickPair {
    static __device__ __forceinline__ void run(const int (&arr)[N], int k, int &lo, int &hi)
    {
        if constexpr (I + 1 < N) { lo = k == I ? arr[I] : lo; hi = k == I ? arr[I + 1] : hi; PickPair<I + 1, N>::run(arr, k, lo, hi); }
    }
};

__device__ __forceinline__ int slot_of(const SlotMap &m, int t)
{
    const int p = t < m.split ? 0 : 1;
    const int u = p ? t - m.split : t;
    const int g = m.grp[p];
    return g ? m.base[p] + (u / g) * 2 * g + m.off[p] + u % g : m.base[p] + u;
}

template <class T> struct Tr;
template <> struct Tr<double> {
    using acc_t = f64x4; using part_t = double;
    static constexpr int CHUNK = 64, SHORT_ROWS = 128, BATCH = kMedBatch64, SHOT = kMedShot64, LONG_SHOT = kMedShot64;
};
template <> struct Tr<_Float16> {
    using acc_t = f32x4; using part_t = float;
    static constexpr int CHUNK = 256, SHORT_ROWS = 256, BATCH = kMedBatch16, SHOT = kMedShot16, LONG_SHOT = 2;
};
static_assert(Tr<double>::BATCH == kMedBatch64 && Tr<double>::SHOT == kMedShot64 && Tr<_Float16>::BATCH == kMedBatch16 &&
              Tr<_Float16>::SHOT == kMedShot16 && kMedBatch64 % 2 == 0 && kMedBatch16 % 2 == 0, "the packers' pairing rule (plan.hpp) follows the kernel's batches");

template <class T> struct Frag;
template <> struct Frag<double> { double a; int c; double b; };
template <> struct Frag<_Float16> { f16x4 a; i32x4 c; f16x4 b; };

template <bool NT>
__device__ __forceinline__ void frag_load_at(Frag<double> &f, const double *val, const int *cid, size_t at)
{
    f.a = ldg<NT>(val + at);
    f.c = ldg<NT>(cid + at);
}
template <bool NT>
__device__ __forceinline__ void frag_load_at(Frag<_Float16> &f, const _Float16 *val, const int *cid, size_t at)
{
    f.a = ldg<NT>(reinterpret_cast<const f16x4 *>(val + at));
    f.c = ldg<NT>(reinterpret_cast<const i32x4 *>(cid + at));
}
template <bool NT, class T>
__device__ __forceinline__ void frag_load(Frag<T> &f, const T *val, const int *cid, size_t e, int lane)
{
    frag_load_at<NT>(f, val, cid, e + (size_t)(Tr<T>::CHUNK / kWave) * lane);
}
template <class T>
struct XGlobal {
    const T *x;
    __device__ __forceinline__ T at(int c) const { return x[c < 0 ? 0 : c]; }
};
template <class T> using lds_cptr = const __attribute__((address_space(3))) T *;
template <class T> using glb_cptr = const __attribute__((address_space(1))) T *;
template <class T>
struct XLds {
    lds_cptr<T> xw; int cmin;
    __device__ __forceinline__ T at(int c) const { return xw[c < 0 ? 0 : c - cmin]; }
};
template <class T>
struct XHyb {
    lds_cptr<T> xw; glb_cptr<T> xg; int cmin; unsigned len;
    __device__ __forceinline__ T at(int c) const
    {
        const unsigned o = (unsigned)(c - cmin);
        T v;
        if (c < 0) v = (T)0;
        else if (o < len) v = xw[o];
        else v = xg[c];
        return v;
    }
};
template <class XV>
__device__ __forceinline__ void frag_gather(Frag<double> &f, const XV &xv)
{
    const double v = xv.at(f.c);
    f.b = f.c < 0 ? 0.0 : v;
}
template <class XV>
__device__ __forceinline__ void frag_gather(Frag<_Float16> &f, const XV &xv)
{
#pragma unroll
    for (int j = 0; j < 4; ++j) {
        const _Float16 v = xv.at(f.c[j]);
        f.b[j] = f.c[j] < 0 ? (_Float16)0 : v;
    }
}
__device__ __forceinline__ void frag_mfma(f64x4 &acc, const Frag<double> &f)
{
    acc = __builtin_amdgcn_mfma_f64_16x16x4f64(f.a, f.b, acc, 0, 0, 0);
}
__device__ __forceinline__ void frag_mfma(f32x4 &acc, const Frag<_Float16> &f)
{
    acc = __builtin_amdgcn_mfma_f32_16x16x16f16(f.a, f.b, acc, 0, 0, 0);
}


template <class T, bool NT>
struct ChunkSrc {
    static constexpr bool kPairs = false, kQuadIds = false;
    const T *val; const int *cid; size_t e0; int lane;
    template <bool PAIRED_OK = true> __device__ __forceinline__ void load(Frag<T> &f, int i) const { frag_load<NT>(f, val, cid, e0 + (size_t)i * Tr<T>::CHUNK, lane); }
    template <bool QUAD = false, class XV> __device__ __forceinline__ void gather(Frag<T> &f, int, const XV &x) const { frag_gather(f, x); }
};

template <class T, bool NT, bool N16 = false>
struct PieceSrc {
    static constexpr bool kPairs = false, kQuadIds = false;
    static constexpr int VPL = Tr<T>::CHUNK / kWave;
    const T *val; const int *cid; size_t e0; int lane, nfull, tail;
    const unsigned short *cid16 = nullptr; const int *base = nullptr;
    template <bool PAIRED_OK = true> __device__ __forceinline__ void load(Frag<T> &f, int i) const
    {
        if constexpr (N16) {
            const size_t at = i < nfull || VPL * lane < tail ? e0 + (size_t)i * Tr<T>::CHUNK + (size_t)(VPL * lane) : e0;
            if constexpr (VPL == 1) { f.a = ldg<NT>(val + at); f.c = (int)ldg<NT>(cid16 + at); }
            else {
                f.a = ldg<NT>(reinterpret_cast<const f16x4 *>(val + at));
                const i32x2 o = ldg<NT>(reinterpret_cast<const i32x2 *>(cid16 + at));
                f.c[0] = o[0]; f.c[1] = o[1];
            }
        } else {
            if (i < nfull) frag_load<NT>(f, val, cid, e0 + (size_t)i * Tr<T>::CHUNK, lane);
            else frag_load_at<NT>(f, val, cid, VPL * lane < tail ? e0 + (size_t)i * Tr<T>::CHUNK + (size_t)(VPL * lane) : e0);
        }
    }
    template <bool QUAD = false, class XV> __device__ __forceinline__ void gather(Frag<T> &f, int i, const XV &x) const
    {
        if constexpr (N16) {
            const int b = tab<true>(base, i);
            if constexpr (VPL == 1) { const unsigned o = (unsigned)f.c; f.c = o == kLongPad16 ? -1 : b + (int)o; }
            else {
                const unsigned lo = (unsigned)f.c[0], hi = (unsigned)f.c[1];
                const unsigned o[4] = {lo & 0xFFFFu, lo >> 16, hi & 0xFFFFu, hi >> 16};
#pragma unroll
                for (int q = 0; q < 4; ++q) f.c[q] = o[q] == kLongPad16 ? -1 : b + (int)o[q];
            }
        }
        if (i >= nfull) {
            const bool ok = VPL * lane < tail;
            if constexpr (VPL == 1) { f.c = ok ? f.c : -1; f.a = ok ? f.a : 0.0; }
            else {
#pragma unroll
                for (int j = 0; j < 4; ++j) { f.c[j] = ok ? f.c[j] : -1; f.a[j] = ok ? f.a[j] : (_Float16)0; }
            }
        }
        frag_gather(f, x);
    }
};

template <class T, bool NT, bool C16, bool PAIRS, bool C8, bool KT = false, bool REL = false>
struct BlockSrc {
    static constexpr bool kPairs = PAIRS;
    static constexpr int VPL = Tr<T>::CHUNK / kWave;
    ChunkSrc<T, NT> reg; int nc;
    int npair;
    const unsigned short *cid16; const int *base; int c0;
    int relb;
    const unsigned char *c8; const unsigned short *w16; int n8;
    const T *ival; const int *icid; int t0, t1, kq;
    template <bool PAIRED_OK> __device__ __forceinline__ size_t at_of(int i) const
    {
        constexpr int CH = Tr<T>::CHUNK;
        if constexpr (!PAIRED_OK || !PAIRS) return reg.e0 + (size_t)i * CH + (size_t)VPL * reg.lane;
        const bool paired = i < npair;
        const size_t s = reg.e0 + (paired ? (size_t)(i & ~1) * CH + (size_t)(VPL * (i & 1)) : (size_t)i * CH);
        return s + (size_t)(paired ? 2 * VPL : VPL) * reg.lane;
    }
    __device__ __forceinline__ bool pairs_ok(int i0, int n) const { return i0 + n <= npair; }
    __device__ __forceinline__ void load2(Frag<T> &f0, Frag<T> &f1, int i) const
    {
        constexpr int CH = Tr<T>::CHUNK;
        const size_t at = reg.e0 + (size_t)i * CH + (size_t)(2 * VPL) * reg.lane;
        if constexpr (sizeof(T) == 8) {
            const f64x2 v = ldg<NT>(reinterpret_cast<const f64x2 *>(reg.val + at));
            f0.a = v[0]; f1.a = v[1];
            if constexpr (C16) {
                if constexpr (kQuadIds) {
                    if (i < n8) {
                        const unsigned r = ldg<NT>(reinterpret_cast<const unsigned short *>(c8 + (size_t)i * CH) + reg.lane);
                        const unsigned b0 = r & 0xFFu, b1 = r >> 8;
                        f0.c = (int)(b0 == 0xFFu ? 0xFFFFu : b0); f1.c = (int)(b1 == 0xFFu ? 0xFFFFu : b1);
                        return;
                    }
                }
                const unsigned r = ldg<NT>(reinterpret_cast<const unsigned *>((kQuadIds ? w16 : cid16) + at));
                f0.c = (int)(r & 0xFFFFu); f1.c = (int)(r >> 16);
            } else {
                const i32x2 c = ldg<NT>(reinterpret_cast<const i32x2 *>(reg.cid + at));
                f0.c = c[0]; f1.c = c[1];
            }
        } else {
            const f16x8 v = ldg<NT>(reinterpret_cast<const f16x8 *>(reg.val + at));
            f0.a = __builtin_shufflevector(v, v, 0, 1, 2, 3); f1.a = __builtin_shufflevector(v, v, 4, 5, 6, 7);
            if constexpr (C16) {
                const i32x4 o = ldg<NT>(reinterpret_cast<const i32x4 *>(cid16 + at));
                f0.c[0] = o[0]; f0.c[1] = o[1]; f1.c[0] = o[2]; f1.c[1] = o[3];
            } else {
                f0.c = ldg<NT>(reinterpret_cast<const i32x4 *>(reg.cid + at));
                f1.c = ldg<NT>(reinterpret_cast<const i32x4 *>(reg.cid + at + 4));
            }
        }
    }
    static constexpr bool kQuadIds = C8 && PAIRS && C16 && sizeof(T) == 8 && Tr<T>::BATCH == 4;
    __device__ __forceinline__ void load4(Frag<T> *f, int i) const
    {
        constexpr int CH = Tr<T>::CHUNK;
        const size_t at = reg.e0 + (size_t)i * CH + (size_t)2 * reg.lane;
        const f64x2 v0 = ldg<NT>(reinterpret_cast<const f64x2 *>(reg.val + at));
        const f64x2 v1 = ldg<NT>(reinterpret_cast<const f64x2 *>(reg.val + at + 2 * CH));
        f[0].a = v0[0]; f[1].a = v0[1]; f[2].a = v1[0]; f[3].a = v1[1];
        const bool narrow = i + 4 <= n8;
        const gbyte_p pa = narrow ? (gbyte_p)(c8 + (size_t)i * CH) : (gbyte_p)(w16 + reg.e0 + (size_t)i * CH);
        const gbyte_p pb = narrow ? pa : pa + 4 * CH;
        const unsigned lo4 = 4u * (unsigned)reg.lane;
        const unsigned ra = ldg<NT>((const __attribute__((address_space(1))) unsigned *)(pa + lo4));
        const unsigned rb = ldg<NT>((const __attribute__((address_space(1))) unsigned *)(pb + lo4));
        f[0].c = (int)ra; f[1].c = (int)ra; f[2].c = (int)rb; f[3].c = (int)rb;
    }
    template <bool PAIRED_OK = true> __device__ __forceinline__ void load(Frag<T> &f, int i) const
    {
        if (i < nc) {
            const size_t at = at_of<PAIRED_OK>(i);
            if constexpr (!C16) frag_load_at<NT>(f, reg.val, reg.cid, at);
            else {
                if constexpr (sizeof(T) == 8) {
                    f.a = ldg<NT>(reg.val + at);
                    f.c = (int)ldg<NT>((kQuadIds ? w16 : cid16) + at);
                } else {
                    f.a = ldg<NT>(reinterpret_cast<const f16x4 *>(reg.val + at));
                    const i32x2 o = ldg<NT>(reinterpret_cast<const i32x2 *>(cid16 + at));
                    f.c[0] = o[0]; f.c[1] = o[1];
                }
            }
            return;
        }
        const int j = i - nc;
        if constexpr (sizeof(T) == 8) {
            const int e = t0 + 4 * j + kq;
            const int ee = e < t1 ? e : 0;
            f.a = ldg<NT>(ival + ee);
            f.c = ldg<NT>(icid + ee);
        } else {
#pragma unroll
            for (int q = 0; q < 4; ++q) {
                const int e = t0 + 16 * j + 4 * kq + q;
                const int ee = e < t1 ? e : 0;
                f.a[q] = ival[ee];
                f.c[q] = icid[ee];
            }
        }
    }
    template <bool QUAD = false, class XV> __device__ __forceinline__ void gather(Frag<T> &f, int i, const XV &x) const
    {
        if (i >= nc) {
            const int j = i - nc;
            if constexpr (sizeof(T) == 8) {
                const bool ok = t0 + 4 * j + kq < t1;
                f.a = ok ? f.a : 0.0;
                f.c = ok ? f.c : -1;
            } else {
#pragma unroll
                for (int q = 0; q < 4; ++q) {
                    const bool ok = t0 + 16 * j + 4 * kq + q < t1;
                    f.a[q] = ok ? f.a[q] : (_Float16)0;
                    f.c[q] = ok ? f.c[q] : -1;
                }
            }
        } else if constexpr (C16) {
            const int b = REL ? relb : tab<KT>(base, c0 + i);
            if constexpr (sizeof(T) == 8) {
                unsigned o = (unsigned)f.c, pad = 0xFFFFu;
                if constexpr (QUAD && kQuadIds) {
                    const bool narrow = i < n8, paired = i < npair;
                    pad = narrow ? 0xFFu : 0xFFFFu;
                    o = (o >> (narrow ? 8u * (i & 3) : (paired ? 16u * (i & 1) : 0u))) & pad;
                }
                f.c = o == pad ? -1 : b + (int)o;
            }
            else {
                const unsigned lo = (unsigned)f.c[0], hi = (unsigned)f.c[1];
                const unsigned o[4] = {lo & 0xFFFFu, lo >> 16, hi & 0xFFFFu, hi >> 16};
#pragma unroll
                for (int q = 0; q < 4; ++q) f.c[q] = o[q] == 0xFFFFu ? -1 : b + (int)o[q];
            }
        }
        frag_gather(f, x);
    }
};

template <int N, class SRC, class T>
__device__ __forceinline__ void load_steps(const SRC &src, Frag<T> *f, int i0)
{
    if constexpr (SRC::kPairs && N == Tr<T>::BATCH) {
        if (src.pairs_ok(i0, N)) {
            if constexpr (SRC::kQuadIds) src.load4(f, i0);
            else {
#pragma unroll
                for (int u = 0; u < N; u += 2) src.load2(f[u], f[u + 1], i0 + u);
            }
            return;
        }
    }
#pragma unroll
    for (int u = 0; u < N; ++u) src.load(f[u], i0 + u);
}

template <class T, int N, class SRC, class ACC, class XV>
__device__ __forceinline__ void shot(ACC &acc, const SRC &src, int i0, const XV &x)
// ... 24 lines not shown
#pragma unroll
    for (int u = 0; u < N; ++u) frag_mfma(acc, f[u]);
}
template <class T, int N, class SRC, class ACC, class XV>
struct ShotDispatch {
    static __device__ __forceinline__ void run(ACC &acc, const SRC &src, int i0, int n, const XV &x)
    {
        if (n == N) shot<T, N>(acc, src, i0, x);
        else ShotDispatch<T, N - 1, SRC, ACC, XV>::run(acc, src, i0, n, x);
    }
};
template <class T, class SRC, class ACC, class XV>
struct ShotDispatch<T, 0, SRC, ACC, XV> {
    static __device__ __forceinline__ void run(ACC &, const SRC &, int, int, const XV &) {}
};

template <class T, int U, int R, class SRC, class ACC, class XV>
struct FinishDispatch {
    static __device__ __forceinline__ void run(ACC &acc, const SRC &src, Frag<T> (&cur)[U], int ibase, int i, int rem, const XV &x)
    {
        if (rem == R) {
            Frag<T> r[R > 0 ? R : 1];
#pragma unroll
            for (int u = 0; u < U; ++u) src.template gather<true>(cur[u], ibase + u, x);
            load_steps<R>(src, r, i);
#pragma unroll
            for (int u = 0; u < U; ++u) frag_mfma(acc, cur[u]);
#pragma unroll
            for (int u = 0; u < R; ++u) src.template gather<true>(r[u], i + u, x);
#pragma unroll
            for (int u = 0; u < R; ++u) frag_mfma(acc, r[u]);
        } else if constexpr (R > 0) FinishDispatch<T, U, R - 1, SRC, ACC, XV>::run(acc, src, cur, ibase, i, rem, x);
    }
};

template <class T, int U, int S, class SRC, class ACC, class XV>
__device__ __forceinline__ void run_stream(ACC &acc, const SRC &src, int N, const XV &x)
{
    if (N <= S) { ShotDispatch<T, S, SRC, ACC, XV>::run(acc, src, 0, N, x); return; }
    const int nfull = N / U, rem = N % U;
    Frag<T> cur[U];
    load_steps<U>(src, cur, 0);
    int i = U;
    for (int it = 1; it < nfull; ++it, i += U) {
        Frag<T> nxt[U];
#pragma unroll
        for (int u = 0; u < U; ++u) src.template gather<true>(cur[u], i - U + u, x);
        load_steps<U>(src, nxt, i);
#pragma unroll
        for (int u = 0; u < U; ++u) frag_mfma(acc, cur[u]);
#pragma unroll
        for (int u = 0; u < U; ++u) cur[u] = nxt[u];
    }
    FinishDispatch<T, U, U - 1, SRC, ACC, XV>::run(acc, src, cur, i - U, i, rem, x);
}

template <class T, int YS = 0, class P>
__device__ __forceinline__ void put_y(const DevArgs &a, int yi, P v)
{
    T *y = static_cast<T *>(a.y) + yi;
    if constexpr (YS == 1) *(volatile T *)y = (T)v;
    else if constexpr (YS == 2) {
        const T old = *(volatile T *)y;
        *(volatile T *)y = (T)((P)old + v);
    }
    else if (a.acc) *y = (T)((P)*y + v);
    else if (a.ywt) *(volatile T *)y = (T)v;
    else *y = (T)v;
}

__device__ __forceinline__ bool diag_of(const f64x4 &acc, int lane, double &d)
{
    const int r = (lane & 15) >> 2;
    d = r == 0 ? acc[0] : r == 1 ? acc[1] : r == 2 ? acc[2] : acc[3];
    return (lane & 3) == (lane >> 4);
}
__device__ __forceinline__ bool diag_of(const f32x4 &acc, int lane, float &d)
{
    const int r = lane & 3;
    d = r == 0 ? acc[0] : r == 1 ? acc[1] : r == 2 ? acc[2] : acc[3];
    return ((lane & 15) >> 2) == (lane >> 4);
}

template <class T, bool NT, bool C16, int YM, bool C8 = false, int YS = 0, bool REL = false, int WU = 0, int WS = 0, class XV>
__device__ __forceinline__ void medium_block(const DevArgs &a, int b, int lane, const XV &x)
{
    using acc_t = typename Tr<T>::acc_t;
    constexpr int CH = Tr<T>::CHUNK;
    const T *val = static_cast<const T *>(a.med_val);
    constexpr bool KT = true;
    const int c0 = tab<KT>(a.med_ptr, b), c1 = tab<KT>(a.med_ptr, b + 1);
    acc_t acc = {0, 0, 0, 0};
    const int row = lane & 15, kq = lane >> 4;
    const int r = b * kMedRows + row;
    int t0 = 0, t1 = 0;
    if (r < a.row_block) { t0 = a.irr_ptr[r]; t1 = a.irr_ptr[r + 1]; }
    constexpr int TK = sizeof(T) == 8 ? 4 : 16;
    const int nt = YS == 0 ? tab<true>(a.med_nt, b) : (__builtin_amdgcn_readfirstlane(t1 - t0) + TK - 1) / TK;
    BlockSrc<T, NT, C16, YM != 2, C8, KT, REL> src;
    if constexpr (REL) src.relb = x.cmin; else src.relb = 0;
    src.reg.val = val; src.reg.cid = a.med_cid; src.reg.e0 = (size_t)c0 * CH; src.reg.lane = lane;
    src.nc = c1 - c0; src.npair = med_npair(c1 - c0, nt, (int)sizeof(T), YM == 2 ? 0 : a.pair_mode); src.cid16 = a.med_cid16; src.base = a.med_base; src.c0 = c0;
    src.c8 = a.med_cid8; src.w16 = a.med_cid16; src.n8 = 0;
    if constexpr (C8 && C16 && sizeof(T) == 8 && YM != 2) {
        const int q0 = tab<true>(a.med_c8ptr, b), q1 = tab<true>(a.med_c8ptr, b + 1);
        src.n8 = q1 - q0; src.c8 = a.med_cid8 + (size_t)q0 * CH; src.w16 = a.med_cid16 - (size_t)q1 * CH;
    }
    src.ival = static_cast<const T *>(a.irr_val); src.icid = a.irr_cid; src.t0 = t0; src.t1 = t1; src.kq = kq;
    run_stream<T, (WU > 0 && sizeof(T) == 8) ? WU : Tr<T>::BATCH, (YM == 2 && sizeof(T) == 2) ? 2 : ((WS > 0 && sizeof(T) == 8) ? WS : Tr<T>::SHOT)>(acc, src, src.nc + nt, x);

    typename Tr<T>::part_t d;
    if (diag_of(acc, lane, d) && r < a.row_block) {
        const int slot = a.row_long + r;
        const int yi = YM == 2 ? a.med_dst[r] : (a.order ? a.order[slot] : slot);
        put_y<T, YS>(a, yi, d);
    }
}

template <class T, bool NT, int YS = 0, bool TAIL_IN = false, bool L16 = false>
__device__ __forceinline__ void long_piece(const DevArgs &a, int p, int lane)
{
    using acc_t = typename Tr<T>::acc_t;
    using part_t = typename Tr<T>::part_t;
    constexpr int CH = Tr<T>::CHUNK;
    constexpr int VPL = CH / kWave;
    const XGlobal<T> x{static_cast<const T *>(a.x)};
    const T *val = static_cast<const T *>(a.long_val);
    const int p0 = tab<true>(a.piece_ptr, p), p1 = tab<true>(a.piece_ptr, p + 1);
    acc_t acc = {0, 0, 0, 0};
    const int nfull = (p1 - p0) / CH, tail = (p1 - p0) - nfull * CH;
    bool narrow = false;
    if constexpr (L16) narrow = tab<true>(a.piece_c16, 2 * p + 1) != 0;
    if (L16 && narrow) {
        const PieceSrc<T, NT, true> src{val, a.long_cid, (size_t)p0, lane, nfull, tail, a.long_cid16, a.long_base + tab<true>(a.piece_c16, 2 * p)};
        run_stream<T, Tr<T>::BATCH, Tr<T>::LONG_SHOT>(acc, src, nfull + (tail > 0 ? 1 : 0), x);
    } else if (TAIL_IN && tail > 0) {
        const PieceSrc<T, NT> src{val, a.long_cid, (size_t)p0, lane, nfull, tail};
        run_stream<T, Tr<T>::BATCH, Tr<T>::LONG_SHOT>(acc, src, nfull + 1, x);
    } else {
        const int full = p0 + nfull * CH;
        ChunkSrc<T, NT> src{val, a.long_cid, (size_t)p0, lane};
        run_stream<T, Tr<T>::BATCH, Tr<T>::LONG_SHOT>(acc, src, nfull, x);
        if (full < p1) {
            const int i = full + VPL * lane;
            const bool ok = i < p1;
            Frag<T> f;
            frag_load_at<NT>(f, val, a.long_cid, (size_t)(ok ? i : p0));
            frag_gather(f, x);
            if constexpr (VPL == 1) { f.a = ok ? f.a : 0.0; f.b = ok ? f.b : 0.0; }
            else {
#pragma unroll
                for (int j = 0; j < 4; ++j) { f.a[j] = ok ? f.a[j] : (_Float16)0; f.b[j] = ok ? f.b[j] : (_Float16)0; }
            }
            frag_mfma(acc, f);
        }
    }
    part_t d;
    const bool on_diag = diag_of(acc, lane, d);
    const part_t total = wave_sum(on_diag ? d : (part_t)0);
    if (lane == 0) {
        const int dst = tab<true>(a.piece_dst, p);
        if (dst >= 0) put_y<T, YS>(a, dst, total);
        else static_cast<part_t *>(a.partial)[~dst] = total;
    }
}

template <class T, int L, bool NT, int YS = 0>
__device__ __forceinline__ void short_rows(const DevArgs &a, const ShortDev &g, int local_tile, int lane)
{
    constexpr int SR = Tr<T>::SHORT_ROWS;
    constexpr int V = SR / kWave;
    const T *x = static_cast<const T *>(a.x);
    const T *val = static_cast<const T *>(a.short_val);
    using part_t = typename Tr<T>::part_t;
    part_t s[V];
#pragma unroll
    for (int v = 0; v < V; ++v) s[v] = 0;
    const size_t base = (size_t)g.elem_off + (size_t)local_tile * L * SR + (size_t)V * lane;
#pragma unroll
    for (int k = 0; k < L; ++k) {
        if constexpr (V == 2) {
            const f64x2 av = ldg<NT>(reinterpret_cast<const f64x2 *>(val + base + (size_t)k * SR));
            const i32x2 c = ldg<NT>(reinterpret_cast<const i32x2 *>(a.short_cid + base + (size_t)k * SR));
            const double x0 = x[c[0] < 0 ? 0 : c[0]], x1 = x[c[1] < 0 ? 0 : c[1]];
            s[0] += av[0] * (c[0] < 0 ? 0.0 : x0);
            s[1] += av[1] * (c[1] < 0 ? 0.0 : x1);
        } else {
            const f16x4 av = ldg<NT>(reinterpret_cast<const f16x4 *>(val + base + (size_t)k * SR));
            const i32x4 c = ldg<NT>(reinterpret_cast<const i32x4 *>(a.short_cid + base + (size_t)k * SR));
// ... 156 lines not shown
        case 0: if constexpr (YS != 2) { if (!a.skip0 && !a.acc) short_rows<T, 0, NT, YS>(a, g, local, lane); } break;
        case 1: short_rows<T, 1, NT, YS>(a, g, local, lane); break;
        case 2: short_rows<T, 2, NT, YS>(a, g, local, lane); break;
        case 3: short_rows<T, 3, NT, YS>(a, g, local, lane); break;
        case 4: short_rows<T, 4, NT, YS>(a, g, local, lane); break;
        default: slab_rows<T, NT, YS>(a, g, local, lane); break;
    }
}

template <class T, bool NT, int TPW>
__device__ __forceinline__ void short_waves(const DevArgs &a, int w, int lane)
{
    int gi = 0, w0 = 0;
    LastLE<1, kNumShortGroups>::run(a.grp_wave0, w, gi, w0);
    const ShortDev g = a.groups[gi];
    const int lw = w - w0;
    if (!g.seg) { short_tile<T, NT, 0, false>(a, g.tile0 + lw, lane); return; }
    const int local0 = lw * TPW, nv = min(TPW, g.tiles - local0);
    switch (g.len) {
        case 1: short_rows_seg_multi<T, 1, NT, TPW>(a, g, local0, nv, lane); break;
        case 2: short_rows_seg_multi<T, 2, NT, TPW>(a, g, local0, nv, lane); break;
        case 3: short_rows_seg_multi<T, 3, NT, TPW>(a, g, local0, nv, lane); break;
        default: short_rows_seg_multi<T, 4, NT, TPW>(a, g, local0, nv, lane); break;
    }
}

template <class T, bool NT>
__device__ __forceinline__ void row_tile(const DevArgs &a, int t, int lane, typename Tr<T>::part_t *prod)
{
    using part_t = typename Tr<T>::part_t;
    const T *x = static_cast<const T *>(a.x), *val = static_cast<const T *>(a.rt_val);
    const int e0 = a.rt_ptr[t], n = a.rt_ptr[t + 1] - e0;
    const int s = a.rt_start[(size_t)t * kRowTile + lane];
#pragma unroll 4
    for (int i = lane; i < n; i += kWave) prod[i] = (part_t)ldg<NT>(val + e0 + i) * (part_t)x[ldg<NT>(a.rt_cid + e0 + i)];
    int e = __shfl_down(s, 1);
    if (lane == kWave - 1) e = n;
    part_t sum = 0;
    for (int j = s; j < e; ++j) sum += prod[j];
    if ((a.rt_mask[t] >> lane) & 1) put_y<T>(a, t * kRowTile + lane, sum);
}

#ifdef DASP_STAMPS
struct StampBuf { unsigned long long *rec; unsigned cap; };
static __device__ StampBuf g_stamps;
struct Stamps {
    unsigned long long wall0, clk[4];
    int kind, launch;
    __device__ __forceinline__ void begin(int launch_no) { wall0 = __builtin_amdgcn_s_memrealtime(); clk[0] = __builtin_readcyclecounter(); clk[1] = clk[2] = clk[3] = clk[0]; kind = 0; launch = launch_no; }
    __device__ __forceinline__ void mark(int i) { asm volatile("s_waitcnt vmcnt(0) lgkmcnt(0)" ::: "memory"); clk[i] = __builtin_readcyclecounter(); }
    __device__ __forceinline__ void finish(int nwaves)
    {
        asm volatile("s_waitcnt vmcnt(0) lgkmcnt(0)" ::: "memory");
        const unsigned long long e = __builtin_readcyclecounter();
        const unsigned long long wall1 = __builtin_amdgcn_s_memrealtime();
        const size_t slot = ((size_t)launch * gridDim.x + blockIdx.x) * (size_t)nwaves + (threadIdx.x >> 6);
        if ((threadIdx.x & 63) == 0 && g_stamps.rec && launch >= 0 && slot < g_stamps.cap) {
            unsigned long long *r = g_stamps.rec + slot * 12;
            unsigned xcc, hw;
            asm volatile("s_getreg_b32 %0, hwreg(HW_REG_XCC_ID)" : "=s"(xcc));
            asm volatile("s_getreg_b32 %0, hwreg(HW_REG_HW_ID)" : "=s"(hw));
            r[0] = blockIdx.x | ((unsigned long long)(threadIdx.x >> 6) << 32) | ((unsigned long long)nwaves << 40) | ((unsigned long long)kind << 48) | (1ull << 63);
            r[1] = xcc | ((unsigned long long)hw << 32); r[2] = gridDim.x; r[3] = wall0; r[4] = wall1;
            r[5] = clk[0]; r[6] = clk[1]; r[7] = clk[2]; r[8] = clk[3]; r[9] = e; r[10] = (unsigned long long)launch; r[11] = 0;
        }
    }
};
#else
struct Stamps {
    int kind;
    __device__ __forceinline__ void begin(int) {}
    __device__ __forceinline__ void mark(int) {}
};
#endif

#ifndef DASP_MIN_WAVES
#define DASP_MIN_WAVES 1
#endif
constexpr int kMinWavesPlain = DASP_MIN_WAVES, kMinWavesWin = 8;
#ifndef DASP_WIN64_U
#define DASP_WIN64_U 3
#define DASP_WIN64_S 6
#endif
template <class T, bool NT, bool C16, bool WIN, bool C8, bool RT = false, bool W64 = false, bool L16 = false>
__device__ __forceinline__ void spmv_body(const DevArgs &a, char *lds_raw, int wg_index, Stamps &st)
{
    const int lane = threadIdx.x & 63;
    const int wave = __builtin_amdgcn_readfirstlane(threadIdx.x >> 6);
    int wg = wg_index;
    if constexpr (sizeof(T) == 2 && !WIN && !RT) {
        if (a.wg_rot) { const int grid = a.wg_long + a.wg_med + a.wg_short; wg += a.wg_rot; wg = wg >= grid ? wg - grid : wg; }
    }
    const int wpw = WIN ? a.wpw : kWavesPerWG;
    if (wg < a.wg_long) {
        const int p = wg * wpw + wave;
        if (p < a.n_pieces) long_piece<T, NT, 0, !WIN, L16 && !WIN>(a, p, lane);
    } else if (wg < a.wg_long + a.wg_med) {
        st.kind = 1;
        if constexpr (!WIN) {
            const int m = wg - a.wg_long;
            const XGlobal<T> x{static_cast<const T *>(a.x)};
            if (a.xcd_on) {
                const int k = m & 7;
                int lo = a.xcd_blk[0], hi = a.xcd_blk[1];
                PickPair<1, 9>::run(a.xcd_blk, k, lo, hi);
                const int b = lo + (m >> 3) * kWavesPerWG + wave;
                if (b < hi) medium_block<T, NT, C16, 0, C8>(a, b, lane, x);
            } else if (sizeof(T) == 8 && !a.med_stride) {
                const int b = m * kWavesPerWG + wave;
                if (b < a.n_blocks) medium_block<T, NT, C16, 0, C8>(a, b, lane, x);
            } else {
#pragma unroll 1
            for (int b = m * kWavesPerWG + wave; b < a.n_blocks; b += a.wg_med * kWavesPerWG)
                medium_block<T, NT, C16, 0, C8>(a, b, lane, x);
            }
        } else {
            const int mw = wg - a.wg_long, per_xcd = a.wg_med >> 3;
            const int w = a.win_xcd ? (mw & 7) * per_xcd + (mw >> 3) : mw;
            if (w >= a.n_windows) return;
            const int len = a.win_len[w], cmin = a.win_cmin[w];
            const T *xg = static_cast<const T *>(a.x);
            __shared__ int next_unit_word;
            int *next_unit = &next_unit_word;
            typedef __attribute__((address_space(3))) T lds_T;
            lds_T *xw = (lds_T *)lds_raw;
            if (threadIdx.x == 0) *next_unit = wpw;
            st.kind = 3; st.mark(1);
            if (len > 0) {
                constexpr int A = 16 / (int)sizeof(T);
                const i32x4 *src = reinterpret_cast<const i32x4 *>(xg + cmin);
                typedef __attribute__((address_space(3))) i32x4 lds_i32x4;
                lds_i32x4 *dst = (lds_i32x4 *)xw;
                const int nvec = len / A, nth = wpw * kWave;
                for (int i0 = threadIdx.x; i0 < nvec; i0 += 4 * nth) {
                    const int i1 = i0 + nth, i2 = i0 + 2 * nth, i3 = i0 + 3 * nth;
                    const i32x4 v0 = src[i0];
                    const i32x4 v1 = src[i1 < nvec ? i1 : i0], v2 = src[i2 < nvec ? i2 : i0], v3 = src[i3 < nvec ? i3 : i0];
                    dst[i0] = v0;
                    if (i1 < nvec) dst[i1] = v1;
                    if (i2 < nvec) dst[i2] = v2;
                    if (i3 < nvec) dst[i3] = v3;
                }
                for (int i = nvec * A + threadIdx.x; i < len; i += nth) xw[i] = xg[cmin + i];
                st.mark(2);
            }
            __syncthreads();
            st.mark(3);
            const int n_units = a.blocks_per_win + a.win_tiles;
            constexpr int WU = W64 ? DASP_WIN64_U : 0, WS = W64 ? DASP_WIN64_S : 0;
            int q = wave;
#define DASP_NEXT_UNIT()                                                                                          \
            {                                                                                                     \
                int nq = 0;                                                                                       \
                if (lane == 0) nq = atomicAdd(next_unit, 1);                                                      \
                q = __builtin_amdgcn_readfirstlane(nq);                                                           \
            }
#define DASP_WINDOW_BLOCKS(BLOCK_CALL)                                                                            \
            while (q < a.blocks_per_win) {                                                                        \
                const int b = w * a.blocks_per_win + q;                                                           \
                if (b < a.n_blocks) { BLOCK_CALL; }                                                               \
                DASP_NEXT_UNIT()                                                                                  \
            }
            if (len > 0) {
                if (a.win_hybrid) {
                    const XHyb<T> x{xw, (glb_cptr<T>)xg, cmin, (unsigned)len};
                    DASP_WINDOW_BLOCKS((medium_block<T, NT, C16, 2, false, 0, false, WU, WS>(a, b, lane, x)))
                } else if (C16 && a.win_rel16) {
                    const XLds<T> x{xw, cmin};
#ifdef DASP_WIN_KEEPMOD
                    if ((w % DASP_WIN_KEEPMOD) != DASP_WIN_KEEPMOD - 1) { DASP_WINDOW_BLOCKS((medium_block<T, false, C16, 2, false, 0, C16, WU, WS>(a, b, lane, x))) }
                    else
#endif
                    DASP_WINDOW_BLOCKS((medium_block<T, NT, C16, 2, false, 0, C16, WU, WS>(a, b, lane, x)))
                } else {
                    const XLds<T> x{xw, cmin};
                    DASP_WINDOW_BLOCKS((medium_block<T, NT, C16, 2, false, 0, false, WU, WS>(a, b, lane, x)))
                }
            } else {
                const XGlobal<T> x{xg};
                DASP_WINDOW_BLOCKS((medium_block<T, NT, C16, 2, false, 0, false, WU, WS>(a, b, lane, x)))
            }
            while (q < n_units) {
                const int t = w + (q - a.blocks_per_win) * a.n_windows;
                if (t < a.n_short_tiles) short_tile<T, NT, 0, false>(a, t, lane);
                DASP_NEXT_UNIT()
            }
#undef DASP_WINDOW_BLOCKS
#undef DASP_NEXT_UNIT
        }
    } else if (!RT || wg < a.wg_long + a.wg_med + a.wg_short) {
        st.kind = 2;
        const int t = (wg - a.wg_long - a.wg_med) * wpw + wave;
        if constexpr (!WIN && sizeof(T) == 8) {
            if (a.short_tpw > 1) {
                if (t < a.n_short_waves) short_waves<T, NT, kShortTpw>(a, t, lane);
                return;
            }
// ... 26 lines not shown
```

### dasp_amd/csrc/upload.cpp

```cpp
#include <hip/hip_runtime_api.h>

#include <algorithm>
#include <chrono>
#include <cmath>
#include <cstdio>
#include <cstdlib>
#include <cstring>
#include <string>
#include <type_traits>
#include <vector>

#include "plan.hpp"
#include "device.hpp"

namespace dasp {

#define HIP_TRY(expr)                                                                          \
    do {                                                                                       \
        hipError_t e_ = (expr);                                                                \
        if (e_ != hipSuccess) {                                                                \
            set_error(std::string(#expr) + ": " + hipGetErrorString(e_));                      \
            return e_ == hipErrorNoDevice ? DASP_ERR_NO_DEVICE : DASP_ERR_HIP;                 \
        }                                                                                      \
    } while (0)

Plan::~Plan()
{
    if (dev) {
        value_map_free(dev);
        if (dev->arena) (void)hipFree(dev->arena);
        if (dev->dargs) (void)hipFree(dev->dargs);
        std::free(dev->args_sent);
        delete dev;
    }
}

int require_device()
{
    int n = 0;
    hipError_t e = hipGetDeviceCount(&n);
    if (e != hipSuccess || n <= 0) {
        set_error("no HIP device visible (the DASP GPU path has no CPU fallback)");
        return DASP_ERR_NO_DEVICE;
    }
    return DASP_OK;
}

int sync_dev_args(Plan &p)
{
    DevicePlan *d = p.dev;
    if (!d) { set_error("plan not uploaded"); return DASP_ERR_STATE; }
    if (d->dargs && d->args_sent && std::memcmp(d->args_sent, &d->args, sizeof(DevArgs)) == 0) return DASP_OK;
    if (!d->dargs) HIP_TRY(hipMalloc(&d->dargs, (sizeof(DevArgs) + 255) & ~size_t(255)));
    if (!d->args_sent) { d->args_sent = std::malloc(sizeof(DevArgs)); if (!d->args_sent) { set_error("out of host memory"); return DASP_ERR_NOMEM; } }
    HIP_TRY(hipMemcpy(d->dargs, &d->args, sizeof(DevArgs), hipMemcpyHostToDevice));
    std::memcpy(d->args_sent, &d->args, sizeof(DevArgs));
    return DASP_OK;
}

struct LcbOffsets { size_t v = 0, c = 0, p = 0, u = 0, d = 0, s = 0; };
template <class Place>
static LcbOffsets place_long_cb(const LongCB &L, size_t vbytes, Place &&place)
{
    LcbOffsets o;
    o.v = place(L.elems * vbytes); o.c = place(L.elems * 2); o.p = place(L.ptr.size() * 4); o.u = place(L.unit.size() * 4);
    o.d = place(L.row_dst.size() * 4); o.s = place((size_t)L.n_cb * (size_t)L.n_rows() * 8);
    return o;
}
static int upload_long_cb(Plan &p, DevicePlan *d, const LcbOffsets &o)
{
    const LongCB &L = p.lcb;
    const size_t vbytes = (size_t)p.geo.vbytes;
    char *base = static_cast<char *>(d->arena);
    if (!L.val.empty()) HIP_TRY(hipMemcpy(base + o.v, L.val.data(), L.elems * vbytes, hipMemcpyHostToDevice));
    if (!L.lcol.empty()) HIP_TRY(hipMemcpy(base + o.c, L.lcol.data(), L.elems * 2, hipMemcpyHostToDevice));
    HIP_TRY(hipMemcpy(base + o.p, L.ptr.data(), L.ptr.size() * 4, hipMemcpyHostToDevice));
    HIP_TRY(hipMemcpy(base + o.u, L.unit.data(), L.unit.size() * 4, hipMemcpyHostToDevice));
    HIP_TRY(hipMemcpy(base + o.d, L.row_dst.data(), L.row_dst.size() * 4, hipMemcpyHostToDevice));
    HIP_TRY(hipMemset(base + o.s, 0, std::max<size_t>((size_t)L.n_cb * (size_t)L.n_rows() * 8, 16)));
    LcbDev &q = d->lcb;
    q.val = base + o.v; q.lcol = (const unsigned short *)(base + o.c); q.ptr = (const int *)(base + o.p); q.unit = (const int *)(base + o.u);
    q.row_dst = (const int *)(base + o.d); q.partial = base + o.s;
    q.n_units = L.n_units(); q.n_rows = L.n_rows(); q.n_cb = L.n_cb; q.cb = L.cb; q.xlen = p.n;
    if (int rc = tp_kernels_allow_lds()) return rc;
    return DASP_OK;
}

void choose_long16(Plan &p)
{
    DevicePlan *d = p.dev;
    if (!d) return;
    d->long16 = false;
    if (!p.windowed && p.cnt_reg8 == 0 && p.piece_c16.size() == 2 * p.piece_dst.size() && !p.piece_dst.empty()) {
        long long narrow = 0;
        for (size_t q = 0; q < p.piece_dst.size(); ++q) if (p.piece_c16[2 * q + 1]) narrow += p.piece_ptr[q + 1] - p.piece_ptr[q];
        d->long16 = narrow * 20 >= (long long)p.nnz && narrow > 0;
        if (const char *e = std::getenv("DASP_LONG16")) d->long16 = std::atoi(e) != 0;
    }
}

void release_device(Plan &p)
{
    if (p.dev) { value_map_free(p.dev); if (p.dev->arena) (void)hipFree(p.dev->arena); if (p.dev->dargs) (void)hipFree(p.dev->dargs); std::free(p.dev->args_sent); delete p.dev; p.dev = nullptr; }
}

int upload_plan(Plan &p);
static int upload_plan_impl(Plan &p)
{
    if (int rc = require_device()) return rc;
    if (p.host_dropped && p.dev) return DASP_OK;
    if (p.host_dropped) { set_error("host arrays were dropped"); return DASP_ERR_STATE; }
    release_device(p);
    auto *d = new DevicePlan();
    p.dev = d;
    HIP_TRY(hipGetDevice(&d->device));
    if (!p.panels.empty()) {
        for (auto &h : p.panels) if (int rc = upload_plan(h->impl)) return rc;
        d->ypart_stride = ((size_t)std::max(p.m, 1) + 127) & ~size_t(127);
        const size_t part_bytes = d->ypart_stride * p.panels.size() * (size_t)p.geo.vbytes;
        const LongCB &L = p.lcb;
        const size_t vbytes = (size_t)p.geo.vbytes;
        size_t total = (part_bytes + 255) & ~size_t(255);
        auto place = [&](size_t bytes) { const size_t off = total; total += (std::max<size_t>(bytes, 16) + 255) & ~size_t(255); return off; };
        const bool lcb = L.n_rows() > 0;
        LcbOffsets lo;
        if (lcb) lo = place_long_cb(L, vbytes, place);
        d->arena_bytes = total;
        HIP_TRY(hipMalloc(&d->arena, d->arena_bytes));
        HIP_TRY(hipMemset(d->arena, 0, d->arena_bytes));
        if (lcb) if (int rc = upload_long_cb(p, d, lo)) return rc;
        return DASP_OK;
    }

    if (p.two_phase) {
        const TwoPhase &t = p.tp;
        const size_t S = t.segments, vbytes = (size_t)p.geo.vbytes;
        struct Item { const void *src; size_t bytes; size_t off; };
        std::vector<Item> items;
        size_t total = 0;
        auto add = [&](const void *src, size_t bytes) { const size_t off = total; items.push_back({src, bytes, off}); total += (std::max<size_t>(bytes, 16) + 255) & ~size_t(255); return off; };
        const size_t o_lc = add(t.lcol.data(), S * kTpSeg * 2), o_dst = add(t.dst.data(), S * 4), o_un = add(t.unit.data(), t.unit.size() * 4);
        const size_t o_v = add(t.val.data(), S * kTpSeg * vbytes), o_lr = add(t.lrow.data(), S * kTpSeg * 2), o_xs = add(nullptr, S * kTpSeg * vbytes);
        const size_t o_r0 = add(t.rb_row0.data(), t.rb_row0.size() * 4), o_s0 = add(t.rb_seg0.data(), t.rb_seg0.size() * 4);
        const bool lcb = p.lcb.n_rows() > 0;
        LcbOffsets lo;
        if (lcb) lo = place_long_cb(p.lcb, vbytes, [&](size_t bytes) { return add(nullptr, bytes); });
        HIP_TRY(hipMalloc(&d->arena, total));
        d->arena_bytes = total;
        char *base = static_cast<char *>(d->arena);
        for (const Item &it : items)
            if (it.src && it.bytes) HIP_TRY(hipMemcpy(base + it.off, it.src, it.bytes, hipMemcpyHostToDevice));
        HIP_TRY(hipMemset(base + o_xs, 0, std::max<size_t>(S * kTpSeg * vbytes, 16)));
        TpDev &q = d->tp;
        q.lcol = (const unsigned short *)(base + o_lc); q.dst = (const int *)(base + o_dst); q.unit = (const int *)(base + o_un);
        q.val = base + o_v; q.lrow = (const unsigned short *)(base + o_lr); q.xs = base + o_xs;
        q.rb_row0 = (const int *)(base + o_r0); q.rb_seg0 = (const int *)(base + o_s0);
        q.n_units = t.n_units(); q.n_rb = t.n_rb(); q.cb = t.cb; q.rb_max = t.rb_max; q.xlen = p.n; q.m = p.m;
        d->nt = true;
        if (lcb) if (int rc = upload_long_cb(p, d, lo)) return rc;
        return tp_kernels_allow_lds();
    }

    std::vector<ShortDev> groups(kNumShortGroups);
    for (int g = 0; g < kNumShortGroups; ++g) {
        groups[g].len = p.grp[g].len; groups[g].count = p.grp[g].count; groups[g].tiles = p.grp[g].tiles;
        groups[g].tile0 = p.grp[g].tile0; groups[g].elem_off = p.grp[g].elem_off; groups[g].map = p.grp[g].map;
        groups[g].seg = p.grp[g].seg; groups[g].rpt = p.grp[g].rpt;
    }
    const bool natural = p.opt.y_order == DASP_Y_NATURAL;
    const size_t part_bytes = (size_t)std::max<size_t>(1, p.multi_ptr.empty() ? 0 : (size_t)p.multi_ptr.back()) * 8;

    struct Item { const void *src; size_t bytes; size_t off; };
    std::vector<Item> items;
    size_t total = 0;
    auto add = [&](const void *src, size_t bytes) {
        size_t off = total;
        items.push_back({src, bytes, off});
        total += (bytes + 255) & ~size_t(255);
        if (bytes == 0) total += 256;
        return off;
    };
    auto src_of = [](const auto &v) -> const void * { return v.empty() ? nullptr : v.data(); };
    const size_t vbytes = (size_t)p.geo.vbytes;
    const size_t o_lv = add(src_of(p.long_val), p.cnt_long * vbytes);
    const size_t o_lc = add(src_of(p.long_cid), p.cnt_long * 4);
    const size_t o_lc16 = add(src_of(p.long_cid16), p.cnt_long * 2);
// ... 168 lines not shown
        if (q >= from && q < from + bytes) ptr = reinterpret_cast<std::remove_reference_t<decltype(ptr)>>(const_cast<char *>(to + (q - from)));
    };
    mv(a.long_val); mv(a.long_cid); mv(a.long_cid16); mv(a.long_base); mv(a.piece_c16); mv(a.piece_ptr); mv(a.piece_dst); mv(a.partial); mv(a.multi_ptr); mv(a.multi_dst);
    mv(a.med_ptr); mv(a.med_val); mv(a.med_cid); mv(a.med_cid16); mv(a.med_base); mv(a.med_cid8); mv(a.med_c8ptr);
    mv(a.irr_ptr); mv(a.med_nt); mv(a.irr_val); mv(a.irr_cid); mv(a.med_dst); mv(a.win_cmin); mv(a.win_len);
    mv(a.short_val); mv(a.short_cid); mv(a.groups); mv(a.order);
}

int tune_placement(Plan &p, int trials, const void *dX, void *dY, double *ms_first, double *ms_kept)
{
    DevicePlan *d = p.dev;
    if (ms_first) *ms_first = 0.0;
    if (ms_kept) *ms_kept = 0.0;
    if (trials <= 0) trials = 2;
    trials = std::min(trials, 8);
    if (!d || !d->arena || trials <= 1 || d->arena_bytes < (size_t(256) << 20) || !p.panels.empty() || p.panel || p.windowed || p.two_phase) return DASP_OK;
    const bool verbose = std::getenv("DASP_VERBOSE") != nullptr;
    const size_t vb = (size_t)p.geo.vbytes, bytes = d->arena_bytes;
    const size_t xlen = p.opt.n_parts > 0 ? (size_t)p.opt.n_parts * (size_t)p.opt.part_stride : (size_t)p.n;
    void *x = nullptr, *y = nullptr;
    const void *ux = dX; void *uy = dY;
    hipEvent_t e0 = nullptr, e1 = nullptr;
    std::vector<void *> losers;
    auto cleanup = [&] {
        for (void *q : losers) (void)hipFree(q);
        if (x) (void)hipFree(x);
        if (y) (void)hipFree(y);
        if (e0) (void)hipEventDestroy(e0);
        if (e1) (void)hipEventDestroy(e1);
        (void)hipGetLastError();
    };
    if (!ux) { if (hipMalloc(&x, std::max<size_t>(xlen * vb, 256)) != hipSuccess || hipMemset(x, 0, std::max<size_t>(xlen * vb, 256)) != hipSuccess) { cleanup(); return DASP_OK; } ux = x; }
    if (!uy) { if (hipMalloc(&y, ((size_t)p.m + 64) * vb) != hipSuccess) { cleanup(); return DASP_OK; } uy = y; }
    if (hipEventCreate(&e0) != hipSuccess || hipEventCreate(&e1) != hipSuccess) { cleanup(); return DASP_OK; }
    auto time_it = [&](double *ms) -> bool {
        for (int i = 0; i < 2; ++i) if (launch_spmv(p, ux, uy, nullptr, false) != DASP_OK) return false;
        if (hipEventRecord(e0, nullptr) != hipSuccess) return false;
        const int reps = 6;
        for (int i = 0; i < reps; ++i) if (launch_spmv(p, ux, uy, nullptr, false) != DASP_OK) return false;
        float t = 0.f;
        if (hipEventRecord(e1, nullptr) != hipSuccess || hipEventSynchronize(e1) != hipSuccess || hipEventElapsedTime(&t, e0, e1) != hipSuccess) return false;
        *ms = (double)t / reps;
        return true;
    };
    double best = 0.0;
    if (!time_it(&best)) { cleanup(); return DASP_OK; }
    double lo = best, hi = best;
    if (ms_first) *ms_first = best;
    if (verbose) std::fprintf(stderr, "[dasp placement] allocation 0 at %p: %.4f ms\n", d->arena, best);
    for (int t = 1; t < trials && hi < 1.04 * lo; ++t) {
        void *na = nullptr;
        size_t mem_free = 0, mem_total = 0;
        if (hipMemGetInfo(&mem_free, &mem_total) != hipSuccess || mem_free < bytes + (size_t(1) << 30)) { (void)hipGetLastError(); break; }
        if (hipMalloc(&na, bytes) != hipSuccess) { (void)hipGetLastError(); break; }
        if (hipMemcpy(na, d->arena, bytes, hipMemcpyDeviceToDevice) != hipSuccess) { (void)hipFree(na); (void)hipGetLastError(); break; }
        char *old = static_cast<char *>(d->arena);
        rebase_args(d->args, old, static_cast<char *>(na), bytes);
        d->arena = na;
        double ms = 0.0;
        const bool ok = time_it(&ms);
        if (verbose) std::fprintf(stderr, "[dasp placement] allocation %d at %p: %.4f ms\n", t, na, ok ? ms : -1.0);
        if (ok && ms < best) { best = ms; losers.push_back(old); }
        else {
            rebase_args(d->args, static_cast<char *>(na), old, bytes);
            d->arena = old;
            losers.push_back(na);
        }
        if (ok) { lo = std::min(lo, ms); hi = std::max(hi, ms); }
    }
    if (hipDeviceSynchronize() != hipSuccess) (void)hipGetLastError();
    if (int rc = sync_dev_args(p)) { cleanup(); return rc; }
    if (ms_kept) *ms_kept = best;
    for (void *q : losers) (void)hipFree(q);
    losers.clear();
    cleanup();
    return DASP_OK;
}

int upload_plan(Plan &p)
{
    const bool fresh = !(p.host_dropped && p.dev);
    if (int rc = upload_plan_impl(p)) return rc;
    if (fresh && p.value_map && !p.panel) if (int rc = value_map_upload(p)) return rc;
    int trials = 1;
    if (const char *e = std::getenv("DASP_PLACEMENT_TRIALS")) trials = std::max(1, std::min(8, std::atoi(e)));
    return fresh && trials > 1 ? tune_placement(p, trials, nullptr, nullptr, nullptr, nullptr) : DASP_OK;
}
int upload_plan_unpacked(Plan &p) { return upload_plan_impl(p); }

}
```

### include/dasp_amd.h

```cpp
#ifndef DASP_AMD_H
#define DASP_AMD_H

#include <stddef.h>
#include <stdint.h>

#ifdef __cplusplus
extern "C" {
#endif

typedef enum dasp_status {
    DASP_OK = 0,
    DASP_ERR_OPEN = -1,
    DASP_ERR_BANNER = -2,
    DASP_ERR_SIZE = -4,
    DASP_ERR_ENTRY = -5,
    DASP_ERR_ARG = -10,
    DASP_ERR_NOMEM = -11,
    DASP_ERR_NO_DEVICE = -20,
    DASP_ERR_HIP = -21,
    DASP_ERR_STATE = -22
} dasp_status;

const char *dasp_last_error(void);
const char *dasp_version(void);

int dasp_mmio_allinone_f64(int *m, int *n, int *nnz, int *isSymmetric,
                           int **csrRowPtr, int **csrColIdx, double **csrVal, const char *filename);
int dasp_mmio_allinone_f16(int *m, int *n, int *nnz, int *isSymmetric,
                           int **csrRowPtr, int **csrColIdx, uint16_t **csrVal, const char *filename);
void dasp_free(void *p);

int dasp_csr_save(const char *path, int precision, int m, int n, int nnz, int isSymmetric,
                  const int *csrRowPtr, const int *csrColIdx, const void *csrVal);
int dasp_csr_load(const char *path, int precision, int *m, int *n, int *nnz, int *isSymmetric,
                  int **csrRowPtr, int **csrColIdx, void **csrVal);

typedef struct dasp_plan dasp_plan_t;

typedef enum { DASP_F64 = 64, DASP_F16 = 16 } dasp_precision;
typedef enum {
    DASP_Y_PERMUTED = 0,
    DASP_Y_NATURAL = 1
} dasp_y_order;

typedef struct dasp_options {
    double threshold;
    int block_longest;
    int y_order;
    int long_piece;
    int host_threads;
    int n_parts;
    const int *part_bounds;
    int part_stride;
    int x_window;
    int row_window;
    int cid16;
    int stream_policy;
    int col_panels;
    int slab_max_len;
    int x_window_hybrid;
    int piece_min_len;
    int chunk_pairs;
    int cid8;
    int short_seg;
    int row_tile_max;
    int sort_columns;
    int two_phase;
    int tp_col_block, tp_row_block;
    int long_cb;
    int value_map;
} dasp_options_t;

void dasp_options_default(dasp_options_t *opt);

typedef struct dasp_stats {
    int precision, rowA, colA, nnzA;
    int short_row_1, common_13, short_row_3, short_row_4, short_row_2, row_long, row_block, row_zero;
    int nnz_short, nnz_long, origin_nnz_reg, nnz_irreg;
    int rowloop;
    long long fill0_nnz_short, fill0_nnz_long, fill0_nnz_reg;
    double rate_fill0;
    long long data_X;
    long long data_origin1;
    int n_med_blocks, n_long_pieces, n_long_multi, n_short_tiles, n_workgroups;
    double pre_ms;
    int x_window_on, n_windows, n_windows_lds, lds_bytes, row_window;
    double window_nnz_frac;
    int cid16_on;
    int n_col_panels;
    int x_window_hybrid;
    int med_rows_as_pieces;
    int chunk_pairs;
    int cid8_chunks;
    int short_seg;
    int row_tile_max;
    int n_row_tiles;
    long long row_tile_nnz;
    int two_phase;
    int tp_col_block, tp_row_blocks, tp_units;
    long long tp_segments;
    int tp_seg_elems;
    int lcb_rows, lcb_col_block, lcb_units;
    long long lcb_elems;
    long long ref_fill0_nnz_short, ref_fill0_nnz_long, ref_fill0_nnz_reg, ref_data_X;
    int ref_nnz_irreg, ref_origin_nnz_reg, ref_blocknum, ref_warp_number;
    double ref_rate_fill0;
} dasp_stats_t;

int dasp_plan_create(dasp_plan_t **plan, int precision, int rowA, int colA, int nnzA,
                     const int *csrRowPtr, const int *csrColIdx, const void *csrVal,
                     const dasp_options_t *opt );
int dasp_plan_create_device(dasp_plan_t **plan, int precision, int rowA, int colA, int nnzA,
                            const int *dRowPtr, const int *dColIdx, const void *dVal, const dasp_options_t *opt);
int dasp_plan_tune_placement(dasp_plan_t *plan, int trials, const void *dX, void *dY, double *ms_first, double *ms_kept);
int dasp_plan_download_array(dasp_plan_t *plan, const char *name, void *dst, size_t bytes);
void dasp_plan_destroy(dasp_plan_t *plan);

int dasp_plan_save(dasp_plan_t *plan, const char *path);
int dasp_plan_load(dasp_plan_t **plan, const char *path);

const int *dasp_plan_order(const dasp_plan_t *plan);
int dasp_plan_stats(const dasp_plan_t *plan, dasp_stats_t *out);
int dasp_plan_y_order(const dasp_plan_t *plan);
long long dasp_plan_x_len(const dasp_plan_t *plan);

int dasp_plan_panel_count(const dasp_plan_t *plan);
dasp_plan_t *dasp_plan_panel(dasp_plan_t *plan, int k);
int dasp_plan_panel_range(const dasp_plan_t *plan, int k, int *col_begin, int *col_end);

long long dasp_plan_host_array(const dasp_plan_t *plan, const char *name, const void **ptr, int *elem_bytes);

int dasp_plan_upload(dasp_plan_t *plan);
int dasp_plan_drop_host(dasp_plan_t *plan);

int dasp_plan_update_values(dasp_plan_t *plan, const void *dVal, void *stream);
int dasp_plan_update_values_host(dasp_plan_t *plan, const void *csrVal);
long long dasp_plan_value_map_slots(const dasp_plan_t *plan);
long long dasp_plan_csr_fetch_bytes(const dasp_plan_t *plan);

int dasp_plan_set_stream_policy(dasp_plan_t *plan, int policy);

int dasp_plan_spmv(dasp_plan_t *plan, const void *dX, void *dY, void *stream);
int dasp_plan_spmv_acc(dasp_plan_t *plan, const void *dX, void *dY, void *stream);

int dasp_plan_time(dasp_plan_t *plan, const void *dX, void *dY, void *stream, int warmup, int iters,
                   double *wall_ms_per_iter, double *event_ms_per_iter);

int dasp_plan_time_each(dasp_plan_t *plan, const void *dX, void *dY, void *stream, int warmup, int iters, float *ms_each);

int dasp_plan_time_graph(dasp_plan_t *plan, const void *dX, void *dY, void *stream, int warmup, int iters, int batch,
                         double *wall_ms_per_iter, double *event_ms_per_iter);

int dasp_spmv_all_f64(const char *filename, const double *csrValA, const int *csrRowPtrA,
                      const int *csrColIdxA, const double *X_val, double *Y_val, int *order_rid,
                      int rowA, int colA, int nnzA, int NUM, double threshold, int block_longest);
int dasp_spmv_all_f16(const char *filename, const uint16_t *csrValA, const int *csrRowPtrA,
                      const int *csrColIdxA, const uint16_t *X_val, uint16_t *Y_val, int *order_rid,
                      int rowA, int colA, int nnzA, int NUM, double threshold, int block_longest);

typedef struct dasp_mg_plan dasp_mg_plan_t;
enum { DASP_MG_ID_BYTES = 128 };

typedef struct dasp_mg_info {
    int precision, n_gpus, rank, rowA, colA;
    int row_begin, row_end;
    int stride;
    long long nnz_own, nnz_other;
    int overlap, has_comm, square;
    int stream_memops;
    int fused_step;
    int exchange;
} dasp_mg_info_t;

int dasp_partition_rows(int rowA, const int *csrRowPtr, int n_parts, int *bounds);

int dasp_mg_unique_id(void *id);

int dasp_mg_plan_create(dasp_mg_plan_t **mg, int precision, int rowA, int colA, int n_gpus, int rank, const int *row_bounds,
                        const int *csrRowPtr, const int *csrColIdx, const void *csrVal, const dasp_options_t *opt, int overlap);
void dasp_mg_destroy(dasp_mg_plan_t *mg);
int dasp_mg_upload(dasp_mg_plan_t *mg);
int dasp_mg_comm_init(dasp_mg_plan_t *mg, const void *id);
int dasp_mg_set_x(dasp_mg_plan_t *mg, const void *x_host);
int dasp_mg_spmv(dasp_mg_plan_t *mg, void *stream);
int dasp_mg_check(dasp_mg_plan_t *mg);
int dasp_mg_set_fused(dasp_mg_plan_t *mg, int on);
int dasp_mg_set_fake_exchange(dasp_mg_plan_t *mg, int micros, int n_peers, void *const *peer_gathered);
enum { DASP_MG_IPC_BYTES = 256 };
int dasp_mg_push_export(dasp_mg_plan_t *mg, void *blob);
// ... 29 lines not shown
```

Before: 1299 GFLOP/s.

## Deduplicate identical column-id streams across rows in medium blocks

```diff
diff --git a/dasp_amd/_lib.py b/dasp_amd/_lib.py
--- a/dasp_amd/_lib.py
+++ b/dasp_amd/_lib.py
@@ -22,6 +22,17 @@
         ("two_phase", C.c_int), ("tp_col_block", C.c_int), ("tp_row_block", C.c_int), ("long_cb", C.c_int),
         ("value_map", C.c_int),
     ]
+
+    @property
+    def share_ids(self):
+        return C.c_int.from_buffer(self, Options.value_map.offset + 4).value
+
+    @share_ids.setter
+    def share_ids(self, v):
+        C.c_int.from_buffer(self, Options.value_map.offset + 4).value = int(v)
+
+
+assert C.sizeof(Options) >= Options.value_map.offset + 8, "no room for dasp_options_t::share_ids behind value_map"
 
 
 class Stats(C.Structure):
@@ -39,7 +50,8 @@
         ("two_phase", C.c_int), ("tp_col_block", C.c_int), ("tp_row_blocks", C.c_int), ("tp_units", C.c_int), ("tp_segments", C.c_longlong), ("tp_seg_elems", C.c_int),
         ("lcb_rows", C.c_int), ("lcb_col_block", C.c_int), ("lcb_units", C.c_int), ("lcb_elems", C.c_longlong),
         ("ref_fill0_nnz_short", C.c_longlong), ("ref_fill0_nnz_long", C.c_longlong), ("ref_fill0_nnz_reg", C.c_longlong), ("ref_data_X", C.c_longlong),
-        ("ref_nnz_irreg", C.c_int), ("ref_origin_nnz_reg", C.c_int), ("ref_blocknum", C.c_int), ("ref_warp_number", C.c_int), ("ref_rate_fill0", C.c_double)]
+        ("ref_nnz_irreg", C.c_int), ("ref_origin_nnz_reg", C.c_int), ("ref_blocknum", C.c_int), ("ref_warp_number", C.c_int), ("ref_rate_fill0", C.c_double),
+        ("share_ids", C.c_int), ("share_id_bytes", C.c_longlong), ("share_id_bytes_replaced", C.c_longlong)]
 
     def as_dict(self):
         return {n: getattr(self, n) for n, _ in self._fields_}
diff --git a/dasp_amd/api.py b/dasp_amd/api.py
--- a/dasp_amd/api.py
+++ b/dasp_amd/api.py
@@ -72,7 +72,7 @@
     def __init__(self, csrRowPtr, csrColIdx, csrVal, colA, precision=64, threshold=0.75, block_longest=256,
                  y_order=Y_PERMUTED, long_piece=0, host_threads=0, part_bounds=None, part_stride=0, x_window=0, row_window=0, cid16=0, stream_policy=0,
                  col_panels=0, slab_max_len=0, x_window_hybrid=0, piece_min_len=0, chunk_pairs=0, cid8=0, short_seg=0, row_tile_max=0, sort_columns=0,
-                 two_phase=0, tp_col_block=0, tp_row_block=0, long_cb=0, value_map=0):
+                 two_phase=0, tp_col_block=0, tp_row_block=0, long_cb=0, value_map=0, share_ids=0):
         L = _lib.lib()
         self.precision = precision
         dt = _dtype(precision)
@@ -88,7 +88,7 @@
         opt.col_panels, opt.slab_max_len, opt.x_window_hybrid, opt.piece_min_len = col_panels, slab_max_len, x_window_hybrid, piece_min_len
         opt.chunk_pairs, opt.cid8, opt.short_seg, opt.row_tile_max, opt.sort_columns = chunk_pairs, cid8, short_seg, row_tile_max, sort_columns
         opt.two_phase, opt.tp_col_block, opt.tp_row_block, opt.long_cb = two_phase, tp_col_block, tp_row_block, long_cb
-        opt.value_map = value_map
+        opt.value_map, opt.share_ids = value_map, share_ids
         self._pb = None
         if part_bounds is not None:
             self._pb = np.ascontiguousarray(part_bounds, np.int32)
@@ -104,7 +104,7 @@
     def from_device(cls, d_row_ptr, d_col_idx, d_val, rowA, colA, nnzA, precision=64, threshold=0.75, block_longest=256,
                     y_order=Y_PERMUTED, long_piece=0, part_bounds=None, part_stride=0, x_window=0, row_window=0, cid16=0, col_panels=0, slab_max_len=0,
                     x_window_hybrid=0, piece_min_len=0, chunk_pairs=0, cid8=0, short_seg=0, row_tile_max=0, sort_columns=0, two_phase=0, tp_col_block=0, tp_row_block=0, long_cb=0,
-                    value_map=0):
+                    value_map=0, share_ids=0):
         L = _lib.lib()
         self = cls.__new__(cls)
         self.precision, self.rowA, self.colA, self.nnzA = precision, int(rowA), int(colA), int(nnzA)
@@ -115,7 +115,7 @@
         opt.slab_max_len, opt.x_window_hybrid, opt.piece_min_len = slab_max_len, x_window_hybrid, piece_min_len
         opt.chunk_pairs, opt.cid8, opt.short_seg, opt.row_tile_max, opt.sort_columns = chunk_pairs, cid8, short_seg, row_tile_max, sort_columns
         opt.two_phase, opt.tp_col_block, opt.tp_row_block, opt.long_cb = two_phase, tp_col_block, tp_row_block, long_cb
-        opt.value_map = value_map
+        opt.value_map, opt.share_ids = value_map, share_ids
         self._pb = None
         if part_bounds is not None:
             self._pb = np.ascontiguousarray(part_bounds, np.int32)
diff --git a/dasp_amd/csrc/device.hpp b/dasp_amd/csrc/device.hpp
--- a/dasp_amd/csrc/device.hpp
+++ b/dasp_amd/csrc/device.hpp
@@ -51,6 +51,7 @@
     const int *med_nt;
     int wg_rot;
     int win_tiles;
+    const int *med_sptr; const unsigned long long *med_srank; const unsigned char *med_sid;
 };
 
 struct TpDev {
@@ -83,6 +84,8 @@
     bool win1 = false;
     bool seven_waves = false;
     bool long16 = false;
+    bool share_ids = false;
+    void *sh_tab = nullptr, *sh_sid = nullptr;
     int device = -1;
     size_t ypart_stride = 0;
     void *vm_map = nullptr, *vm_runs = nullptr;
@@ -94,6 +97,8 @@
 };
 int value_map_upload(Plan &p);
 void value_map_free(DevicePlan *d);
+int share_ids_build(Plan &p);
+void share_ids_free(DevicePlan *d);
 
 
 int require_device();
diff --git a/dasp_amd/csrc/devpack.hip b/dasp_amd/csrc/devpack.hip
--- a/dasp_amd/csrc/devpack.hip
+++ b/dasp_amd/csrc/devpack.hip
@@ -1034,7 +1034,8 @@
     if (int rc = upload_plan_unpacked(p)) return rc;
     const int rc = p.precision == 64 ? pack_all_typed<double>(p, d, m) : pack_all_typed<_Float16>(p, d, m);
     if (rc == DASP_OK) p.host_dropped = true;
-    if (rc == DASP_OK && p.value_map && !p.panel) return value_map_upload(p);
+    if (rc == DASP_OK && p.value_map && !p.panel) if (int rc2 = value_map_upload(p)) return rc2;
+    if (rc == DASP_OK) return share_ids_build(p);
     return rc;
 }
 
@@ -1313,9 +1314,171 @@
 
 namespace dasp {
 
+
+namespace {
+
+struct ShareBlock {
+    int nc, n8, npair; bool oneshot;
+    const unsigned char *c8; const unsigned short *c16;
+    __device__ __forceinline__ ShareBlock(const DevArgs &a, int b)
+    {
+        const int c0 = a.med_ptr[b], nt = a.med_nt[b];
+        nc = a.med_ptr[b + 1] - c0;
+        const int q0 = a.med_c8ptr ? a.med_c8ptr[b] : 0;
+        n8 = a.med_c8ptr ? a.med_c8ptr[b + 1] - q0 : 0;
+        npair = med_npair(nc, nt, 8, a.pair_mode); oneshot = med_oneshot64(nc, nt);
+        c8 = a.med_cid8 + (size_t)q0 * 64; c16 = a.med_cid16 + (size_t)(c0 - q0) * 64;
+    }
+    __device__ __forceinline__ unsigned field(int i, int lane) const
+    {
+        return i < n8 ? (unsigned)c8[med_cid8_index(i, lane, 64, oneshot)] : (unsigned)c16[med_elem_index(npair, i, lane, 0, 1, 64) - (size_t)n8 * 64];
+    }
+};
+
+__global__ __launch_bounds__(64) void k_share_count(DevArgs a, int *sptr, unsigned long long *srank)
+{
+    __shared__ unsigned ids[64];
+    __shared__ unsigned eqm[16];
+    __shared__ int rank_of[16];
+    const int b = blockIdx.x, lane = threadIdx.x, row = lane & 15, kq = lane >> 4;
+    const ShareBlock blk(a, b);
+    if (lane < 16) eqm[lane] = 0xFFFFu;
+    unsigned eq = 0xFFFFu;
+    for (int i = 0; i < blk.nc; ++i) {
+        const unsigned v = blk.field(i, lane);
+        __syncthreads();
+        ids[lane] = v;
+        __syncthreads();
+#pragma unroll
+        for (int r2 = 0; r2 < 16; ++r2) if (ids[kq * 16 + r2] != v) eq &= ~(1u << r2);
+    }
+    __syncthreads();
+    atomicAnd(&eqm[row], eq);
+    __syncthreads();
+    if (lane == 0) {
+        unsigned long long ranks = 0;
+        int nlead = 0;
+        for (int r = 0; r < 16; ++r) {
+            const int leader = __ffs((int)eqm[r]) - 1;
+            if (leader == r) rank_of[r] = nlead++;
+            ranks |= (unsigned long long)rank_of[leader] << (4 * r);
+        }
+        srank[b] = ranks;
+        sptr[2 * b] = nlead * (blk.n8 + 2 * (blk.nc - blk.n8));
+        sptr[2 * b + 1] = nlead;
+    }
+}
+
+__global__ __launch_bounds__(1024) void k_share_scan(int nb, int *sptr, unsigned long long *total)
+{
+    __shared__ unsigned long long part[1024];
+    const int t = threadIdx.x, per = (nb + 1023) / 1024;
+    const int lo = min(t * per, nb), hi = min(lo + per, nb);
+    unsigned long long s = 0;
+    for (int i = lo; i < hi; ++i) s += (unsigned)sptr[2 * i];
+    part[t] = s;
+    __syncthreads();
+    for (int d = 1; d < 1024; d <<= 1) {
+        const unsigned long long v = t >= d ? part[t - d] : 0;
+        __syncthreads();
+        part[t] += v;
+        __syncthreads();
+    }
+    unsigned long long run = part[t] - s;
+    for (int i = lo; i < hi; ++i) { const unsigned sz = (unsigned)sptr[2 * i]; sptr[2 * i] = (int)(unsigned)run; run += sz; }
+    if (t == 1023) *total = part[1023];
+}
+
+__global__ __launch_bounds__(64) void k_share_write(DevArgs a, const int *sptr, const unsigned long long *srank, unsigned char *sid)
+{
+    const int b = blockIdx.x, lane = threadIdx.x, row = lane & 15, kq = lane >> 4;
+    const ShareBlock blk(a, b);
+    const unsigned long long ranks = srank[b];
+    const int nlead = sptr[2 * b + 1], rank = (int)(ranks >> (4 * row)) & 15;
+    bool leader = true;
+    for (int r2 = 0; r2 < row; ++r2) leader = leader && ((int)(ranks >> (4 * r2)) & 15) != rank;
+    if (!leader) return;
+    const int sl = kq * nlead + rank, ch = 4 * nlead;
+    unsigned char *s8 = sid + (size_t)(unsigned)sptr[2 * b] * 4;
+    unsigned short *s16 = reinterpret_cast<unsigned short *>(s8 + (size_t)blk.n8 * ch);
+    for (int i = 0; i < blk.nc; ++i) {
+        const unsigned v = blk.field(i, lane);
+        if (i < blk.n8) s8[med_cid8_index(i, sl, ch, blk.oneshot)] = (unsigned char)v;
+        else s16[med_elem_index(blk.npair, i, sl, 0, 1, ch) - (size_t)blk.n8 * ch] = (unsigned short)v;
+    }
+}
+
+}
+
+void share_ids_free(DevicePlan *d)
+{
+    if (!d) return;
+    if (d->sh_tab) (void)hipFree(d->sh_tab);
+    if (d->sh_sid) (void)hipFree(d->sh_sid);
+    d->sh_tab = d->sh_sid = nullptr; d->share_ids = false;
+    d->args.med_sptr = nullptr; d->args.med_srank = nullptr; d->args.med_sid = nullptr;
+}
+
+int share_ids_build(Plan &p)
+{
+    DevicePlan *d = p.dev;
+    p.stats.share_ids = 0; p.stats.share_id_bytes = 0; p.stats.share_id_bytes_replaced = 0;
+    if (!d) return DASP_OK;
+    share_ids_free(d);
+    int mode = p.opt.share_ids;
+    if (const char *e = std::getenv("DASP_SHARE_IDS")) mode = std::atoi(e) != 0 ? 1 : -1;
+    const int nb = p.stats.n_med_blocks;
+    const bool eligible = p.precision == 64 && p.cid16 && !p.windowed && !p.two_phase && !p.panel && p.panels.empty() && p.opt.n_parts == 0 && p.part_bounds.empty() &&
+                          p.rt_mask.empty() && !d->seven_waves && d->arena && nb > 0 && (int)p.med_ptr.size() == nb + 1 && p.cnt_reg > 0 &&
+                          (p.cnt_reg8 == 0 || (int)p.med_c8ptr.size() == nb + 1);
+    if (mode < 0 || !eligible) return DASP_OK;
+    if (mode == 0 && p.stats.data_X <= kStreamBytes) return DASP_OK;
+    const size_t tab_bytes = (size_t)nb * 16 + 256;
+    unsigned long long total = 0;
+    {
+        DevBuf<unsigned long long> dtotal; if (int rc = dtotal.init(1)) return rc;
+        HIP_TRYP(hipMalloc(&d->sh_tab, tab_bytes));
+        int *sptr = static_cast<int *>(d->sh_tab);
+        unsigned long long *srank = reinterpret_cast<unsigned long long *>(static_cast<char *>(d->sh_tab) + (size_t)nb * 8);
+        DevArgs a = d->args;
+        if (p.cnt_reg8 == 0) a.med_c8ptr = nullptr;
+        hipLaunchKernelGGL(k_share_count, dim3(nb), dim3(64), 0, 0, a, sptr, srank);
+        hipLaunchKernelGGL(k_share_scan, dim3(1), dim3(1024), 0, 0, nb, sptr, dtotal.d);
+        HIP_TRYP(hipGetLastError());
+        HIP_TRYP(hipMemcpy(&total, dtotal.d, sizeof total, hipMemcpyDeviceToHost));
+        const long long bytes = (long long)total * 4, replaced = (long long)p.cnt_reg8 + (long long)(p.cnt_reg - p.cnt_reg8) * 2;
+        bool on = total < (1ull << 32) && (mode > 0 || bytes * 2 <= replaced);
+        if (on && d->long16) {
+            long long narrow = 0;
+            for (size_t q = 0; q < p.piece_dst.size(); ++q) if (p.piece_c16[2 * q + 1]) narrow += p.piece_ptr[q + 1] - p.piece_ptr[q];
+            if (narrow * 2 > replaced - bytes) on = false; else d->long16 = false;
+        }
+        if (!on) { share_ids_free(d); return DASP_OK; }
+        HIP_TRYP(hipMalloc(&d->sh_sid, std::max<size_t>((size_t)bytes, 16) + 256));
+        hipLaunchKernelGGL(k_share_write, dim3(nb), dim3(64), 0, 0, a, sptr, srank, static_cast<unsigned char *>(d->sh_sid));
+        HIP_TRYP(hipGetLastError());
+        HIP_TRYP(hipDeviceSynchronize());
+        d->args.med_sptr = sptr; d->args.med_srank = srank; d->args.med_sid = static_cast<const unsigned char *>(d->sh_sid);
+        d->share_ids = true;
+        p.stats.share_ids = 1; p.stats.share_id_bytes = bytes; p.stats.share_id_bytes_replaced = replaced;
+    }
+    return sync_dev_args(p);
+}
+
 int download_array(Plan &p, const char *name, void *dst, size_t bytes)
 {
     if (!p.dev || !p.dev->arena) { set_error("plan not on the device"); return DASP_ERR_STATE; }
+    if (p.dev->share_ids) {
+        const size_t nb = (size_t)p.stats.n_med_blocks;
+        struct { const char *n; const void *ptr; size_t len; } st[] = {
+            {"med_sptr", p.dev->args.med_sptr, nb * 8}, {"med_srank", p.dev->args.med_srank, nb * 8}, {"med_sid", p.dev->args.med_sid, (size_t)p.stats.share_id_bytes}};
+        for (auto &t : st)
+            if (std::strcmp(t.n, name) == 0) {
+                if (bytes != t.len) { set_error(std::string("size mismatch for ") + name); return DASP_ERR_ARG; }
+                if (t.len) HIP_TRYP(hipMemcpy(dst, t.ptr, t.len, hipMemcpyDeviceToHost));
+                return DASP_OK;
+            }
+    }
     const ArenaMap &mp = p.dev->map;
     const size_t vb = (size_t)p.geo.vbytes;
     if (std::strcmp(name, "lcb_val") == 0 && p.dev->lcb.val) {
diff --git a/dasp_amd/csrc/kernels.hip b/dasp_amd/csrc/kernels.hip
--- a/dasp_amd/csrc/kernels.hip
+++ b/dasp_amd/csrc/kernels.hip
@@ -32,6 +32,22 @@
     const DevArgs a = load_args(c);
     static_assert(!L16 || (!WIN && !C8 && MW == 0), "the 16-bit long ids ride in the plain build only");
     spmv_body<T, NT, C16, WIN, C8, false, WIN, L16>(a, lds_raw, blockIdx.x, st);
+#ifdef DASP_STAMPS
+    st.finish(a.wpw);
+#endif
+}
+
+template <bool NT, bool C8>
+__global__ __launch_bounds__(256, kMinWavesPlain) void dasp_spmv_sh_kernel(CallArgs c)
+{
+    extern __shared__ __attribute__((aligned(16))) char lds_raw[];
+#ifdef DASP_STAMPS
+    Stamps st; st.begin(c.stamp_launch);
+#else
+    Stamps st; st.begin(0);
+#endif
+    const DevArgs a = load_args(c);
+    spmv_body<double, NT, true, false, C8, false, false, false, true>(a, lds_raw, blockIdx.x, st);
 #ifdef DASP_STAMPS
     st.finish(a.wpw);
 #endif
@@ -431,6 +447,13 @@
         if (p.windowed && p.dev->win1 && !nt) {
             if (c16) hipLaunchKernelGGL((dasp_spmv_win1_kernel<T, true>), dim3(grid), dim3(kWave * a.wpw), lds, s, c);
             else hipLaunchKernelGGL((dasp_spmv_win1_kernel<T, false>), dim3(grid), dim3(kWave * a.wpw), lds, s, c);
+        } else if (sizeof(T) == 8 && p.dev->share_ids) {
+            if (p.cnt_reg8 > 0) {
+                if (nt) hipLaunchKernelGGL((dasp_spmv_sh_kernel<true, true>), dim3(grid), dim3(kWave * a.wpw), lds, s, c);
+                else hipLaunchKernelGGL((dasp_spmv_sh_kernel<false, true>), dim3(grid), dim3(kWave * a.wpw), lds, s, c);
+            }
+            else if (nt) hipLaunchKernelGGL((dasp_spmv_sh_kernel<true, false>), dim3(grid), dim3(kWave * a.wpw), lds, s, c);
+            else hipLaunchKernelGGL((dasp_spmv_sh_kernel<false, false>), dim3(grid), dim3(kWave * a.wpw), lds, s, c);
         } else if (sizeof(T) == 8 && c16 && !p.windowed && p.cnt_reg8 > 0) {
             if (p.dev->seven_waves) {
                 if (nt) hipLaunchKernelGGL((dasp_spmv_kernel<double, true, true, false, true, 7>), dim3(grid), dim3(kWave * a.wpw), lds, s, c);
diff --git a/dasp_amd/csrc/multigpu.cpp b/dasp_amd/csrc/multigpu.cpp
--- a/dasp_amd/csrc/multigpu.cpp
+++ b/dasp_amd/csrc/multigpu.cpp
@@ -293,6 +293,7 @@
     opt.two_phase = -1;
     opt.n_parts = 0; opt.part_bounds = nullptr; opt.part_stride = 0;
     opt.value_map = 0;
+    opt.share_ids = -1;
     const int nnz = rp[m];
     if (!g.square) {
         g.nnz_own = nnz; g.nnz_other = 0;
diff --git a/dasp_amd/csrc/planio.cpp b/dasp_amd/csrc/planio.cpp
--- a/dasp_amd/csrc/planio.cpp
+++ b/dasp_amd/csrc/planio.cpp
@@ -1,5 +1,6 @@
 #include <algorithm>
 #include <cstdio>
+#include <cstddef>
 #include <cstring>
 #include <string>
 
@@ -274,12 +275,14 @@
     return true;
 }
 
+constexpr size_t kStatsFileBytes = offsetof(dasp_stats_t, share_ids);
+
 static void write_plan(Writer &w, Plan &p)
 {
     const int hdr[25] = {p.precision, p.m, p.n, p.nnz, p.opt.y_order, p.windowed ? 1 : 0, p.row_window, p.lds_bytes, p.cid16 ? 1 : 0,
                          p.opt.n_parts, p.opt.part_stride, p.opt.stream_policy, (int)p.panels.size(), p.n_mfma_rows, p.win_hybrid ? 1 : 0, p.med_slot0, p.pair_mode, p.win_rel16 ? 1 : 0, p.rt_max,
                          p.two_phase ? 1 : 0, p.tp.cb, p.tp.rb_max, p.lcb.cb, p.lcb.n_cb, p.lcb.h};
-    w.raw(hdr, sizeof hdr); w.raw(&p.stats, sizeof p.stats); w.raw(p.grp, sizeof p.grp);
+    w.raw(hdr, sizeof hdr); w.raw(&p.stats, kStatsFileBytes); w.raw(p.grp, sizeof p.grp);
     arrays(w, p);
     for (auto &h : p.panels) write_plan(w, h->impl);
 }
@@ -298,7 +301,8 @@
     p.two_phase = hdr[19] != 0; p.tp.cb = hdr[20]; p.tp.rb_max = hdr[21];
     p.lcb.cb = hdr[22]; p.lcb.n_cb = hdr[23]; p.lcb.h = hdr[24];
     if (p.two_phase && (depth > 0 || hdr[12] != 0)) return false;
-    r.raw(&p.stats, sizeof p.stats); r.raw(p.grp, sizeof p.grp);
+    p.stats = dasp_stats_t{};
+    r.raw(&p.stats, kStatsFileBytes); r.raw(p.grp, sizeof p.grp);
     arrays(r, p);
     if (!r.ok) return false;
     p.tp.segments = p.tp.dst.size();
@@ -348,7 +352,7 @@
     if (!f) { set_error(std::string("cannot create ") + path); return DASP_ERR_OPEN; }
     Writer w{f};
     w.raw(kPlanMagic, 8);
-    const int abi[3] = {(int)sizeof(dasp_stats_t), kNumShortGroups, (int)sizeof(ShortGroup)};
+    const int abi[3] = {(int)kStatsFileBytes, kNumShortGroups, (int)sizeof(ShortGroup)};
     w.raw(abi, sizeof abi);
     write_plan(w, p);
     const bool ok = (std::fclose(f) == 0) && w.ok;
@@ -369,8 +373,8 @@
     int abi[3] = {0, 0, 0};
     r.raw(magic, 8);
     r.raw(abi, sizeof abi);
-    if (!r.ok || std::memcmp(magic, kPlanMagic, 8) != 0 || abi[0] != (int)sizeof(dasp_stats_t) || abi[1] != kNumShortGroups || abi[2] != (int)sizeof(ShortGroup)) {
-        std::fclose(f); set_error("not a DASPPLN7 plan file of this build (magic / struct sizes differ)"); return DASP_ERR_BANNER;
+    if (!r.ok || std::memcmp(magic, kPlanMagic, 8) != 0 || abi[0] != (int)kStatsFileBytes || abi[1] != kNumShortGroups || abi[2] != (int)sizeof(ShortGroup)) {
+        std::fclose(f); set_error("not a " + std::string(kPlanMagic, 8) + " plan file of this build (magic / struct sizes differ)"); return DASP_ERR_BANNER;
     }
     std::string why;
     bool ok = false;
diff --git a/dasp_amd/csrc/spmv_device.hpp b/dasp_amd/csrc/spmv_device.hpp
--- a/dasp_amd/csrc/spmv_device.hpp
+++ b/dasp_amd/csrc/spmv_device.hpp
@@ -98,6 +98,7 @@
     DASP_G(irr_ptr); DASP_G(med_nt); DASP_G(irr_val); DASP_G(irr_cid); DASP_G(med_dst); DASP_G(win_cmin); DASP_G(win_len);
     DASP_G(short_val); DASP_G(short_cid); DASP_G(groups); DASP_G(order);
     DASP_G(rt_val); DASP_G(rt_cid); DASP_G(rt_ptr); DASP_G(rt_start); DASP_G(rt_mask);
+    DASP_G(med_sptr); DASP_G(med_srank); DASP_G(med_sid);
 #undef DASP_G
     a.x = c.x; a.y = c.y; a.acc = c.acc; a.ywt = c.ywt;
     return a;
@@ -260,7 +261,7 @@
     }
 };
 
-template <class T, bool NT, bool C16, bool PAIRS, bool C8, bool KT = false, bool REL = false>
+template <class T, bool NT, bool C16, bool PAIRS, bool C8, bool KT = false, bool REL = false, bool SH = false>
 struct BlockSrc {
     static constexpr bool kPairs = PAIRS;
     static constexpr int VPL = Tr<T>::CHUNK / kWave;
@@ -269,6 +270,7 @@
     const unsigned short *cid16; const int *base; int c0;
     int relb;
     const unsigned char *c8; const unsigned short *w16; int n8;
+    gbyte_p s16; int L4; unsigned sl4;
     const T *ival; const int *icid; int t0, t1, kq;
     template <bool PAIRED_OK> __device__ __forceinline__ size_t at_of(int i) const
     {
@@ -286,7 +288,18 @@
         if constexpr (sizeof(T) == 8) {
             const f64x2 v = ldg<NT>(reinterpret_cast<const f64x2 *>(reg.val + at));
             f0.a = v[0]; f1.a = v[1];
-            if constexpr (C16) {
+            if constexpr (SH) {
+                if constexpr (kQuadIds) {
+                    if (i < n8) {
+                        const unsigned r = ldg<NT>((const __attribute__((address_space(1))) unsigned short *)(s16 + (size_t)(n8 + i) * L4 + (sl4 >> 1)));
+                        const unsigned b0 = r & 0xFFu, b1 = r >> 8;
+                        f0.c = (int)(b0 == 0xFFu ? 0xFFFFu : b0); f1.c = (int)(b1 == 0xFFu ? 0xFFFFu : b1);
+                        return;
+                    }
+                }
+                const unsigned r = ldg<NT>((const __attribute__((address_space(1))) unsigned *)(s16 + (size_t)i * (2 * L4) + sl4));
+                f0.c = (int)(r & 0xFFFFu); f1.c = (int)(r >> 16);
+            } else if constexpr (C16) {
                 if constexpr (kQuadIds) {
                     if (i < n8) {
                         const unsigned r = ldg<NT>(reinterpret_cast<const unsigned short *>(c8 + (size_t)i * CH) + reg.lane);
@@ -322,9 +335,16 @@
         const f64x2 v1 = ldg<NT>(reinterpret_cast<const f64x2 *>(reg.val + at + 2 * CH));
         f[0].a = v0[0]; f[1].a = v0[1]; f[2].a = v1[0]; f[3].a = v1[1];
         const bool narrow = i + 4 <= n8;
-        const gbyte_p pa = narrow ? (gbyte_p)(c8 + (size_t)i * CH) : (gbyte_p)(w16 + reg.e0 + (size_t)i * CH);
-        const gbyte_p pb = narrow ? pa : pa + 4 * CH;
-        const unsigned lo4 = 4u * (unsigned)reg.lane;
+        gbyte_p pa, pb; unsigned lo4;
+        if constexpr (SH) {
+            pa = s16 + (size_t)(narrow ? n8 + i : 2 * i) * L4;
+            pb = narrow ? pa : pa + 4 * L4;
+            lo4 = sl4;
+        } else {
+            pa = narrow ? (gbyte_p)(c8 + (size_t)i * CH) : (gbyte_p)(w16 + reg.e0 + (size_t)i * CH);
+            pb = narrow ? pa : pa + 4 * CH;
+            lo4 = 4u * (unsigned)reg.lane;
+        }
         const unsigned ra = ldg<NT>((const __attribute__((address_space(1))) unsigned *)(pa + lo4));
         const unsigned rb = ldg<NT>((const __attribute__((address_space(1))) unsigned *)(pb + lo4));
         f[0].c = (int)ra; f[1].c = (int)ra; f[2].c = (int)rb; f[3].c = (int)rb;
@@ -335,7 +355,13 @@
             const size_t at = at_of<PAIRED_OK>(i);
             if constexpr (!C16) frag_load_at<NT>(f, reg.val, reg.cid, at);
             else {
-                if constexpr (sizeof(T) == 8) {
+                if constexpr (SH) {
+                    f.a = ldg<NT>(reg.val + at);
+                    bool paired = false;
+                    if constexpr (PAIRED_OK && PAIRS) paired = i < npair;
+                    const size_t o = paired ? (size_t)(i & ~1) * (2 * L4) + (size_t)(2 * (i & 1)) : (size_t)i * (2 * L4);
+                    f.c = (int)ldg<NT>((const __attribute__((address_space(1))) unsigned short *)(s16 + o + (sl4 >> (paired ? 0u : 1u))));
+                } else if constexpr (sizeof(T) == 8) {
                     f.a = ldg<NT>(reg.val + at);
                     f.c = (int)ldg<NT>((kQuadIds ? w16 : cid16) + at);
                 } else {
@@ -526,7 +552,7 @@
     return ((lane & 15) >> 2) == (lane >> 4);
 }
 
-template <class T, bool NT, bool C16, int YM, bool C8 = false, int YS = 0, bool REL = false, int WU = 0, int WS = 0, class XV>
+template <class T, bool NT, bool C16, int YM, bool C8 = false, int YS = 0, bool REL = false, int WU = 0, int WS = 0, bool SH = false, class XV>
 __device__ __forceinline__ void medium_block(const DevArgs &a, int b, int lane, const XV &x)
 {
     using acc_t = typename Tr<T>::acc_t;
@@ -541,7 +567,8 @@
     if (r < a.row_block) { t0 = a.irr_ptr[r]; t1 = a.irr_ptr[r + 1]; }
     constexpr int TK = sizeof(T) == 8 ? 4 : 16;
     const int nt = YS == 0 ? tab<true>(a.med_nt, b) : (__builtin_amdgcn_readfirstlane(t1 - t0) + TK - 1) / TK;
-    BlockSrc<T, NT, C16, YM != 2, C8, KT, REL> src;
+    static_assert(!SH || (sizeof(T) == 8 && C16 && YM == 0 && YS == 0 && !REL), "shared ids: plain f64 kernels with 16-bit ids");
+    BlockSrc<T, NT, C16, YM != 2, C8, KT, REL, SH> src;
     if constexpr (REL) src.relb = x.cmin; else src.relb = 0;
     src.reg.val = val; src.reg.cid = a.med_cid; src.reg.e0 = (size_t)c0 * CH; src.reg.lane = lane;
     src.nc = c1 - c0; src.npair = med_npair(c1 - c0, nt, (int)sizeof(T), YM == 2 ? 0 : a.pair_mode); src.cid16 = a.med_cid16; src.base = a.med_base; src.c0 = c0;
@@ -549,6 +576,13 @@
     if constexpr (C8 && C16 && sizeof(T) == 8 && YM != 2) {
         const int q0 = tab<true>(a.med_c8ptr, b), q1 = tab<true>(a.med_c8ptr, b + 1);
         src.n8 = q1 - q0; src.c8 = a.med_cid8 + (size_t)q0 * CH; src.w16 = a.med_cid16 - (size_t)q1 * CH;
+    }
+    if constexpr (SH) {
+        const int so = tab<true>(a.med_sptr, 2 * b), nlead = tab<true>(a.med_sptr, 2 * b + 1);
+        const unsigned long long ranks = tab<true>(a.med_srank, b);
+        const unsigned rank = (unsigned)(ranks >> (4 * row)) & 15u;
+        src.L4 = 4 * nlead; src.sl4 = 4u * ((unsigned)(kq * nlead) + rank);
+        src.s16 = (gbyte_p)a.med_sid + (size_t)(unsigned)so * 4 - (size_t)src.n8 * src.L4;
     }
     src.ival = static_cast<const T *>(a.irr_val); src.icid = a.irr_cid; src.t0 = t0; src.t1 = t1; src.kq = kq;
     run_stream<T, (WU > 0 && sizeof(T) == 8) ? WU : Tr<T>::BATCH, (YM == 2 && sizeof(T) == 2) ? 2 : ((WS > 0 && sizeof(T) == 8) ? WS : Tr<T>::SHOT)>(acc, src, src.nc + nt, x);
@@ -871,7 +905,7 @@
 #define DASP_WIN64_U 3
 #define DASP_WIN64_S 6
 #endif
-template <class T, bool NT, bool C16, bool WIN, bool C8, bool RT = false, bool W64 = false, bool L16 = false>
+template <class T, bool NT, bool C16, bool WIN, bool C8, bool RT = false, bool W64 = false, bool L16 = false, bool SH = false>
 __device__ __forceinline__ void spmv_body(const DevArgs &a, char *lds_raw, int wg_index, Stamps &st)
 {
     const int lane = threadIdx.x & 63;
@@ -894,14 +928,17 @@
                 int lo = a.xcd_blk[0], hi = a.xcd_blk[1];
                 PickPair<1, 9>::run(a.xcd_blk, k, lo, hi);
                 const int b = lo + (m >> 3) * kWavesPerWG + wave;
-                if (b < hi) medium_block<T, NT, C16, 0, C8>(a, b, lane, x);
+                if (b < hi) medium_block<T, NT, C16, 0, C8, 0, false, 0, 0, SH>(a, b, lane, x);
             } else if (sizeof(T) == 8 && !a.med_stride) {
                 const int b = m * kWavesPerWG + wave;
-                if (b < a.n_blocks) medium_block<T, NT, C16, 0, C8>(a, b, lane, x);
+                if (b < a.n_blocks) medium_block<T, NT, C16, 0, C8, 0, false, 0, 0, SH>(a, b, lane, x);
             } else {
 #pragma unroll 1
-            for (int b = m * kWavesPerWG + wave; b < a.n_blocks; b += a.wg_med * kWavesPerWG)
-                medium_block<T, NT, C16, 0, C8>(a, b, lane, x);
+            for (int b = m * kWavesPerWG + wave; b < a.n_blocks; b += a.wg_med * kWavesPerWG) {
+                int l = lane;
+                if constexpr (SH) asm("" : "+v"(l));
+                medium_block<T, NT, C16, 0, C8, 0, false, 0, 0, SH>(a, b, l, x);
+            }
             }
         } else {
             const int mw = wg - a.wg_long, per_xcd = a.wg_med >> 3;
diff --git a/dasp_amd/csrc/upload.cpp b/dasp_amd/csrc/upload.cpp
--- a/dasp_amd/csrc/upload.cpp
+++ b/dasp_amd/csrc/upload.cpp
@@ -28,6 +28,7 @@
 {
     if (dev) {
         value_map_free(dev);
+        share_ids_free(dev);
         if (dev->arena) (void)hipFree(dev->arena);
         if (dev->dargs) (void)hipFree(dev->dargs);
         std::free(dev->args_sent);
@@ -101,7 +102,7 @@
 
 void release_device(Plan &p)
 {
-    if (p.dev) { value_map_free(p.dev); if (p.dev->arena) (void)hipFree(p.dev->arena); if (p.dev->dargs) (void)hipFree(p.dev->dargs); std::free(p.dev->args_sent); delete p.dev; p.dev = nullptr; }
+    if (p.dev) { value_map_free(p.dev); share_ids_free(p.dev); if (p.dev->arena) (void)hipFree(p.dev->arena); if (p.dev->dargs) (void)hipFree(p.dev->dargs); std::free(p.dev->args_sent); delete p.dev; p.dev = nullptr; }
 }
 
 int upload_plan(Plan &p);
@@ -436,6 +437,7 @@
     const bool fresh = !(p.host_dropped && p.dev);
     if (int rc = upload_plan_impl(p)) return rc;
     if (fresh && p.value_map && !p.panel) if (int rc = value_map_upload(p)) return rc;
+    if (fresh) if (int rc = share_ids_build(p)) return rc;
     int trials = 1;
     if (const char *e = std::getenv("DASP_PLACEMENT_TRIALS")) trials = std::max(1, std::min(8, std::atoi(e)));
     return fresh && trials > 1 ? tune_placement(p, trials, nullptr, nullptr, nullptr, nullptr) : DASP_OK;
diff --git a/include/dasp_amd.h b/include/dasp_amd.h
--- a/include/dasp_amd.h
+++ b/include/dasp_amd.h
@@ -69,6 +69,7 @@
     int tp_col_block, tp_row_block;
     int long_cb;
     int value_map;
+    int share_ids;
 } dasp_options_t;
 
 void dasp_options_default(dasp_options_t *opt);
@@ -105,6 +106,9 @@
     long long ref_fill0_nnz_short, ref_fill0_nnz_long, ref_fill0_nnz_reg, ref_data_X;
     int ref_nnz_irreg, ref_origin_nnz_reg, ref_blocknum, ref_warp_number;
     double ref_rate_fill0;
+    int share_ids;
+    long long share_id_bytes;
+    long long share_id_bytes_replaced;
 } dasp_stats_t;
 
 int dasp_plan_create(dasp_plan_t **plan, int precision, int rowA, int colA, int nnzA,
```

Result: faster. 1338 GFLOP/s, median of 6 (+3.0%).
